# Parsoa/SVDSS

Measured on AMD Instinct MI355X. Metric: reads/sec through search+call, 30x HiFi 15 kb reads vs 3 Gb ref, 1/2/4/8 GPU, higher is better.
Workload: dtype int64

## Files before the change

svdss_amd/csrc/call_dp.hip:

```cpp
#include <hip/hip_runtime.h>

#include <cstdint>
#include <algorithm>
#include <chrono>
#include <cstdio>
#include <cstring>
#include <new>
#include <string>
#include <vector>

#include "../../include/svdss_hip.h"
#include "call_streams.h"
#include "dev_arena.h"
#include "hip_check.h"

#define DP_NEG (-0x20000000)
#define DP_THREADS 256

struct GapModel { int q, e, q2, e2; };

__device__ __forceinline__ int dp_gap(int l, const GapModel& g) {
  const int a = g.q + l * g.e, b = g.q2 + l * g.e2;
  return a < b ? a : b;
}

struct AlnPair {
  int64_t q_off, t_off;
  int64_t bnd_off;
  int64_t dir_off;
  int64_t cig_off;
  int32_t ql, tl;
  int32_t slot;
  int32_t waves;
};

__device__ __forceinline__ int dp_shr1(int x) {
  return __builtin_amdgcn_update_dpp(x, x, 0x138, 0xf, 0xf, false);
}

template <int W>
__global__ void __launch_bounds__(64 * W) align_wave_kernel(
    const AlnPair* pairs, const uint8_t* qsyms, const uint8_t* tsyms, int m, const int8_t* mat_g,
    GapModel gm, int32_t* ws, uint8_t* dirs, uint32_t* cigars, int32_t* scores, int32_t* n_cigar, int32_t* abort_flag) {
  const AlnPair P = pairs[blockIdx.x];
  const int ql = P.ql, tl = P.tl;
  const int lane = threadIdx.x & 63, wave = threadIdx.x >> 6;
  const int Wp = W > 1 ? P.waves : 1, NB = Wp + 1;
  if (wave >= Wp) return;
  if (ql <= 0 || tl <= 0) {
    if (lane == 0) { scores[P.slot] = 0; n_cigar[P.slot] = 0; }
    return;
  }
  __shared__ volatile int32_t prog[W + 1];
  __shared__ int32_t s_score;
  const uint8_t* q = qsyms + P.q_off;
  const uint8_t* t = tsyms + P.t_off;
  uint8_t* dir = dirs + P.dir_off;
  const int bstride = ql + 64;
  int32_t* bnd = ws + P.bnd_off;
  {
    int32_t* b0 = bnd + (int64_t)(NB - 1) * 3 * bstride;
    for (int j = threadIdx.x; j < ql; j += 64 * Wp) { b0[j] = -dp_gap(j + 1, gm); b0[bstride + j] = DP_NEG; b0[2 * bstride + j] = DP_NEG; }
    if ((int)threadIdx.x < NB) prog[threadIdx.x] = (int)threadIdx.x == NB - 1 ? ql : 0;
    __builtin_amdgcn_fence(__ATOMIC_RELEASE, "workgroup");
  }
  __syncthreads();
  const int n_stripes = (tl + 63) >> 6;
  int32_t final_score = 0;
  bool aborted = false;
  for (int s = wave; s < n_stripes && !aborted; s += Wp) {
    const int in_slot = (s + NB - 1) % NB, out_slot = s % NB;
    const int32_t* bin = bnd + (int64_t)in_slot * 3 * bstride;
    int32_t* bout = bnd + (int64_t)out_slot * 3 * bstride;
    if (W > 1 && lane == 0) prog[out_slot] = (s + 1) << 20;
    const int i = (s << 6) + lane;
    const bool row_ok = i < tl;
    const int rows = tl - (s << 6) < 64 ? tl - (s << 6) : 64;
    const bool writes_bnd = lane == 63 && s + 1 < n_stripes;
    uint64_t rowbits = 0;
    {
      const int ti = row_ok ? t[i] : 0;
      for (int k = 0; k < m; ++k) rowbits |= (uint64_t)(uint8_t)mat_g[ti * m + k] << (8 * k);
    }
    int32_t Hl = -dp_gap(i + 1, gm), Fl = DP_NEG, F2l = DP_NEG;
    int32_t Hout = 0, Eout = DP_NEG, E2out = DP_NEG;
    int32_t Hd = 0;
    int qcur = 0;
    const int n_steps = ql + rows - 1;
    int32_t nH = 0, nE = 0, nE2 = 0;
    int nq = 0;
    auto fetch = [&](int tau0) {
      const int jj = tau0 + lane;
      const bool in = jj < ql;
      nq = in ? q[jj] : 0;
      if (W > 1 && Wp > 1) {
        const int need = tau0 + 64 < ql ? tau0 + 64 : ql;
        int polls = 0;
        for (;;) {
          const int32_t v = prog[in_slot];
          if ((v >> 20) == s && (v & 0xFFFFF) >= need) break;
          if (++polls > (1 << 22)) { aborted = true; break; }
          __builtin_amdgcn_s_sleep(2);
        }
        if (aborted) { nH = 0; nE = 0; nE2 = 0; return; }
        __builtin_amdgcn_fence(__ATOMIC_ACQUIRE, "workgroup");
        nH = in ? __hip_atomic_load(&bin[jj], __ATOMIC_RELAXED, __HIP_MEMORY_SCOPE_WORKGROUP) : 0;
        nE = in ? __hip_atomic_load(&bin[bstride + jj], __ATOMIC_RELAXED, __HIP_MEMORY_SCOPE_WORKGROUP) : 0;
        nE2 = in ? __hip_atomic_load(&bin[2 * bstride + jj], __ATOMIC_RELAXED, __HIP_MEMORY_SCOPE_WORKGROUP) : 0;
      } else {
        nH = in ? bin[jj] : 0; nE = in ? bin[bstride + jj] : 0; nE2 = in ? bin[2 * bstride + jj] : 0;
      }
    };
    fetch(0);
    uint8_t* dcell = dir + (int64_t)(s << 6) * tl + i;
    for (int tau0 = 0; tau0 < n_steps && !aborted; tau0 += 64) {
      asm volatile("" : "+v"(nq), "+v"(nH), "+v"(nE), "+v"(nE2));
      const int qblk = nq;
      const int32_t bH = nH, bE = nE, bE2 = nE2;
      if (tau0 + 64 < n_steps) fetch(tau0 + 64);
      const int kmax = n_steps - tau0 < 64 ? n_steps - tau0 : 64;
      for (int k = 0; k < kmax; ++k) {
        const int tau = tau0 + k;
        const int qs = __builtin_amdgcn_readlane(qblk, k);
        const int32_t hb = __builtin_amdgcn_readlane(bH, k), eb = __builtin_amdgcn_readlane(bE, k),
                      e2b = __builtin_amdgcn_readlane(bE2, k);
        qcur = dp_shr1(qcur);
        int32_t Hu = dp_shr1(Hout), Eu = dp_shr1(Eout), E2u = dp_shr1(E2out);
        if (lane == 0) { qcur = qs; Hu = hb; Eu = eb; E2u = e2b; }
        const int j = tau - lane;
        if (row_ok && j >= 0 && j < ql) {
          const int32_t hdiag = j == 0 ? (i == 0 ? 0 : -dp_gap(i, gm)) : Hd;
          const int32_t Ein = (Hu - gm.q > Eu ? Hu - gm.q : Eu) - gm.e;
          const int32_t E2in = (Hu - gm.q2 > E2u ? Hu - gm.q2 : E2u) - gm.e2;
          const int32_t Fin = (Hl - gm.q > Fl ? Hl - gm.q : Fl) - gm.e;
          const int32_t F2in = (Hl - gm.q2 > F2l ? Hl - gm.q2 : F2l) - gm.e2;
          int32_t z = hdiag + (int32_t)(int8_t)(rowbits >> (8 * qcur));
          uint32_t d = 0;
          if (Ein > z) { d = 1; z = Ein; }
          if (Fin > z) { d = 2; z = Fin; }
          if (E2in > z) { d = 3; z = E2in; }
          if (F2in > z) { d = 4; z = F2in; }
          if (Ein > z - gm.q) d |= 0x08;
          if (Fin > z - gm.q) d |= 0x10;
          if (E2in > z - gm.q2) d |= 0x20;
          if (F2in > z - gm.q2) d |= 0x40;
          *dcell = (uint8_t)d;
          Hout = z; Eout = Ein; E2out = E2in;
          Hl = z; Fl = Fin; F2l = F2in;
          if (writes_bnd) { bout[j] = z; bout[bstride + j] = Ein; bout[2 * bstride + j] = E2in; }
          if (i == tl - 1 && j == ql - 1) final_score = z;
        }
        Hd = Hu;
        dcell += tl;
      }
      if (W > 1 && Wp > 1 && s + 1 < n_stripes) {
        __builtin_amdgcn_fence(__ATOMIC_RELEASE, "workgroup");
        const int done = tau0 + kmax - 63;
        if (lane == 63) prog[out_slot] = ((s + 1) << 20) | (done < 0 ? 0 : done > ql ? ql : done);
      }
    }
    if (W == 1 || Wp == 1) __syncthreads();
    else if (s + 1 < n_stripes) { __builtin_amdgcn_fence(__ATOMIC_RELEASE, "workgroup"); if (lane == 63) prog[out_slot] = ((s + 1) << 20) | ql; }
    if (s == n_stripes - 1) {
      const int owner = (tl - 1) & 63;
      final_score = __builtin_amdgcn_readlane(final_score, owner);
      if (lane == 0) s_score = final_score;
    }
  }
  if (aborted && lane == 0) atomicExch(abort_flag, 1);
  __syncthreads();
  if (wave != 0) return;
  final_score = s_score;
  {
    if (lane == 0) scores[P.slot] = final_score;
    uint32_t* cg = cigars + P.cig_off;
    int n = 0, i = tl - 1, j = ql - 1, state = 0;
    uint32_t cur_op = 0xffffffffu, cur_len = 0;
    auto push = [&](uint32_t op, uint32_t len) {
      if (op == cur_op) { cur_len += len; return; }
      if (cur_op != 0xffffffffu) { if (lane == 0) cg[n] = (cur_len << 4) | cur_op; ++n; }
      cur_op = op; cur_len = len;
    };
    int i0 = -(1 << 28), j0 = 0;
    uint32_t win = 0;
    while (i >= 0 && j >= 0) {
      int k = i0 - i, d = j - (j0 - k);
      if (k < 0 || k > 63 || d < 0 || d > 3) {
        i0 = i; j0 = j - 1; k = 0; d = 1;
        const int ii = i0 - lane;
        const int64_t jj = (int64_t)j0 - lane;
        win = 0;
        if (ii >= 0) {
#pragma unroll
          for (int x = 0; x < 4; ++x) {
            const int64_t c = jj + x;
            if (c >= 0 && c < ql) win |= (uint32_t)dir[(int64_t)(ii + c) * tl + ii] << (8 * x);
          }
        }
        asm volatile("" : "+v"(win));
      }
      const uint32_t tmp = ((uint32_t)__builtin_amdgcn_readlane((int)win, k) >> (8 * d)) & 0xffu;
      if (state == 0) state = tmp & 7;
      else if (!((tmp >> (state + 2)) & 1)) state = 0;
      if (state == 0) state = tmp & 7;
      if (state == 0) { push(0, 1); --i; --j; }
      else if (state == 1 || state == 3) { push(2, 1); --i; }
      else { push(1, 1); --j; }
    }
    if (i >= 0) push(2, (uint32_t)(i + 1));
    if (j >= 0) push(1, (uint32_t)(j + 1));
    if (cur_op != 0xffffffffu) { if (lane == 0) cg[n] = (cur_len << 4) | cur_op; ++n; }
    if (lane == 0) n_cigar[P.slot] = n;
  }
}

__device__ __forceinline__ void dp_lds_barrier() {
  __builtin_amdgcn_fence(__ATOMIC_RELEASE, "workgroup", "local");
  __builtin_amdgcn_s_barrier();
  __builtin_amdgcn_fence(__ATOMIC_ACQUIRE, "workgroup", "local");
}

struct LcsPair {
  int64_t a_off, b_off, ws_off;
  int32_t la, lb;
};

template <bool LDS>
__global__ void __launch_bounds__(DP_THREADS) lcs_ratio_kernel(const LcsPair* pairs, const uint8_t* as,
                                                              const uint8_t* bs, int32_t* ws,
                                                              int64_t* lcs_out, double* ratio_out) {
  extern __shared__ int32_t dp_lds[];
  const LcsPair P = pairs[blockIdx.x];
  const int la = P.la, lb = P.lb;
  int64_t lcs = 0;
  if (la > 0 && lb > 0) {
    const uint8_t* a = as + P.a_off;
    const uint8_t* b = bs + P.b_off;
    const int stride = la + 1;
    int32_t* buf = LDS ? dp_lds : ws + P.ws_off;
    if (LDS) {
      uint8_t* sa = (uint8_t*)(dp_lds + 3 * stride);
      uint8_t* sb = sa + la;
      for (int x = threadIdx.x; x < la; x += DP_THREADS) sa[x] = a[x];
      for (int x = threadIdx.x; x < lb; x += DP_THREADS) sb[x] = b[x];
      a = sa;
      b = sb;
      __syncthreads();
    }
    const int n_diag = la + lb - 1;
    for (int r = 0; r < n_diag; ++r) {
      const int32_t* Lm1 = buf + ((r + 2) % 3) * stride;
      const int32_t* Lm2 = buf + ((r + 1) % 3) * stride;
      int32_t* Lc = buf + (r % 3) * stride;
      const int ilo = r - (lb - 1) > 0 ? r - (lb - 1) : 0;
      const int ihi = r < la - 1 ? r : la - 1;
      for (int i = ilo + (int)threadIdx.x; i <= ihi; i += DP_THREADS) {
        const int j = r - i;
        const int32_t diag = (i > 0 && j > 0) ? Lm2[i - 1] : 0;
        const int32_t up = i > 0 ? Lm1[i - 1] : 0;
        const int32_t left = j > 0 ? Lm1[i] : 0;
        Lc[i] = a[i] == b[j] ? diag + 1 : (up > left ? up : left);
      }
      if (LDS) dp_lds_barrier(); else __syncthreads();
    }
    lcs = buf[((n_diag - 1) % 3) * stride + la - 1];
  }
  if (threadIdx.x == 0) {
    const int64_t maximum = (int64_t)la + lb;
    const int64_t dist = maximum - 2 * lcs;
    const double norm_dist = maximum ? (double)dist / (double)maximum : 0.0;
    const double norm_sim = 1.0 - norm_dist;
    lcs_out[blockIdx.x] = lcs;
    ratio_out[blockIdx.x] = norm_sim * 100.0;
  }
}

__global__ void __launch_bounds__(64) lcs_bits_kernel(const LcsPair* pairs, const uint8_t* as, const uint8_t* bs,
                                                      const uint8_t* sym_id, int64_t* lcs_out, double* ratio_out) {
  __shared__ unsigned long long pm[8][64];
  const LcsPair P = pairs[blockIdx.x];
  const int lane = threadIdx.x;
  const bool swap = P.la > P.lb;
  const uint8_t* pat = swap ? bs + P.b_off : as + P.a_off;
  const uint8_t* txt = swap ? as + P.a_off : bs + P.b_off;
  const int m = swap ? P.lb : P.la, n = swap ? P.la : P.lb;
  int64_t lcs = 0;
  if (m > 0) {
    unsigned long long mk[8] = {0, 0, 0, 0, 0, 0, 0, 0};
    for (int i = 0; i < 64; ++i) {
      const int pos = 64 * lane + i;
      const int id = pos < m ? (int)sym_id[pat[pos]] : 255;
#pragma unroll
      for (int k = 0; k < 8; ++k) mk[k] |= (unsigned long long)(id == k) << i;
    }
#pragma unroll
    for (int k = 0; k < 8; ++k) pm[k][lane] = mk[k];
    __syncthreads();
    unsigned long long V = ~0ull;
    for (int j0 = 0; j0 < n; j0 += 64) {
      const int tid = j0 + lane < n ? (int)sym_id[txt[j0 + lane]] : 255;
      const int cnt = n - j0 < 64 ? n - j0 : 64;
      int id = __builtin_amdgcn_readlane(tid, 0);
      unsigned long long cur = id < 8 ? pm[id][lane] : 0ull;
      for (int t = 0; t < cnt; ++t) {
        const int idn = __builtin_amdgcn_readlane(tid, t + 1 < cnt ? t + 1 : t);
        const unsigned long long nxt = idn < 8 ? pm[idn][lane] : 0ull;
        const unsigned long long U = V & cur;
        unsigned long long sum = V + U;
        const unsigned long long gen = __ballot(sum < V), pass = __ballot(sum == ~0ull);
        const unsigned long long carry = (pass + (gen << 1)) ^ pass;
        sum += (carry >> lane) & 1ull;
        V = sum | (V - U);
        cur = nxt;
      }
    }
    const int valid = m - 64 * lane;
    const unsigned long long vm = valid >= 64 ? ~0ull : valid <= 0 ? 0ull : ((1ull << valid) - 1);
    int z = (int)__popcll(~V & vm);
    for (int o = 32; o > 0; o >>= 1) z += __shfl_xor(z, o, 64);
    lcs = z;
  }
  if (lane == 0) {
    const int64_t maximum = (int64_t)P.la + P.lb;
    const int64_t dist = maximum - 2 * lcs;
    const double norm_dist = maximum ? (double)dist / (double)maximum : 0.0;
    const double norm_sim = 1.0 - norm_dist;
    lcs_out[blockIdx.x] = lcs;
    ratio_out[blockIdx.x] = norm_sim * 100.0;
  }
}


struct svdss_aln_batch {
  int64_t n_pairs = 0;
  int64_t total_cigar = 0;
  int64_t cells = 0;
  double kernel_ms = 0.0;
  int64_t info[4] = {0, 0, 0, 0};
  std::vector<int32_t> scores;
  std::vector<int64_t> n_cigar;
  std::vector<uint32_t> cigar;
  int device = -1;
  DevArena arena;
};

namespace {
struct DevMem {
  void* p = nullptr;
  ~DevMem() { if (p) (void)hipFree(p); }
  int alloc(size_t bytes) {
    HIPCHK(hipMalloc(&p, bytes ? bytes : 16));
    return SVDSS_OK;
  }
};
}

extern "C" int svdss_align_global_batch(const uint8_t* queries, const int64_t* q_off,
                                        const uint8_t* targets, const int64_t* t_off, int64_t n_pairs,
                                        int32_t m, const int8_t* mat, int32_t gapo, int32_t gape,
                                        int32_t gapo2, int32_t gape2, int32_t device,
                                        svdss_aln_batch_t** out) {
  if (!out || n_pairs < 0 || m < 1 || m > 8 || !mat || device < 0) return SVDSS_EINVAL;
  if (n_pairs > 0 && (!queries || !q_off || !targets || !t_off)) return SVDSS_EINVAL;
  HIPCHK(hipSetDevice(device));
  svdss_aln_batch* b = *out ? *out : new (std::nothrow) svdss_aln_batch();
  if (!b) return SVDSS_ENOMEM;
  *out = b;
  b->n_pairs = n_pairs;
  b->total_cigar = 0;
  b->cells = 0;
  b->kernel_ms = 0.0;
  b->info[0] = b->info[1] = b->info[2] = b->info[3] = 0;
  b->scores.assign((size_t)n_pairs, 0);
  b->n_cigar.assign((size_t)n_pairs, 0);
  b->cigar.clear();
  if (n_pairs == 0) return SVDSS_OK;
  for (int64_t i = 0; i < n_pairs; ++i) {
    const int64_t ql = q_off[i + 1] - q_off[i], tl = t_off[i + 1] - t_off[i];
    if (ql < 0 || tl < 0) return SVDSS_EINVAL;
    if (ql >= (1 << 28) || tl >= (1 << 28)) return SVDSS_ERANGE;
  }
  const int64_t qtot = q_off[n_pairs] - q_off[0], ttot = t_off[n_pairs] - t_off[0];
  if (b->device != device) {
    b->arena.drop();
    b->device = device;
  }
  CallStreamLease lease;
  HIPCHK(lease.acquire(device));
  const hipStream_t st = lease.get();
  const GapModel gm{gapo, gape, gapo2, gape2};
  hipEvent_t ev0, ev1;
  HIPCHK(hipEventCreate(&ev0));
  HIPCHK(hipEventCreate(&ev1));
  int64_t dir_budget = (int64_t)24 << 30;
  {
    size_t free_b = 0, total_b = 0;
    if (hipMemGetInfo(&free_b, &total_b) == hipSuccess)
      dir_budget = std::min<int64_t>(dir_budget, (int64_t)((free_b + b->arena.cap) / 2));
    if (dir_budget < ((int64_t)1 << 30)) dir_budget = (int64_t)1 << 30;
    if (getenv("SVDSS_ALIGN_DIR_MB") && atoll(getenv("SVDSS_ALIGN_DIR_MB")) > 0) dir_budget = atoll(getenv("SVDSS_ALIGN_DIR_MB")) << 20;
  }
  std::vector<int32_t> h_nc((size_t)n_pairs, 0);
  std::vector<std::pair<int64_t, int64_t>> cig_at((size_t)n_pairs);
  std::vector<std::vector<uint32_t>> chunk_cigs;
  int64_t start = 0;
  const int ALN_W = getenv("SVDSS_ALIGN_WAVES") && atoi(getenv("SVDSS_ALIGN_WAVES")) == 8 ? 8 : 4;
  const int64_t aln_frac = getenv("SVDSS_ALIGN_FRAC") && atoll(getenv("SVDSS_ALIGN_FRAC")) > 0 ? atoll(getenv("SVDSS_ALIGN_FRAC")) : 8;
  int64_t max_cells = 0;
  for (int64_t i = 0; i < n_pairs; ++i) max_cells = std::max(max_cells, (q_off[i + 1] - q_off[i]) * (t_off[i + 1] - t_off[i]));
  bool multi = !(getenv("SVDSS_ALIGN_WAVES") && atoi(getenv("SVDSS_ALIGN_WAVES")) <= 1);
  auto waves_of = [&](int64_t ql, int64_t tl) {
    if (!multi || tl < 8 * 64 || ql >= (1 << 20)) return 1;
    return (ql * tl * aln_frac >= max_cells || n_pairs < 2048) ? ALN_W : 1;
  };
  while (start < n_pairs) {
    std::vector<AlnPair> hp;
    int64_t ws = 0, dirb = 0, cig = 0, end = start;
    bool any_multi = false;
    while (end < n_pairs) {
      const int64_t ql = q_off[end + 1] - q_off[end], tl = t_off[end + 1] - t_off[end];
      const int64_t need = (ql + tl) * tl;
      if (end > start && dirb + need > dir_budget) break;
      AlnPair a;
      memset(&a, 0, sizeof a);
      a.q_off = q_off[end] - q_off[0];
      a.t_off = t_off[end] - t_off[0];
      a.bnd_off = ws;
      a.dir_off = dirb;
      a.cig_off = cig;
      a.ql = (int32_t)ql;
      a.tl = (int32_t)tl;
      a.slot = (int32_t)(end - start);
      a.waves = waves_of(ql, tl);
      any_multi = any_multi || a.waves > 1;
      hp.push_back(a);
      cig_at[(size_t)end] = {cig, (int64_t)chunk_cigs.size()};
      ws += 3 * (a.waves + 1) * (ql + 64);
      dirb += need;
      cig += ql + tl + 2;
      b->cells += ql * tl;
      ++end;
    }
    const int64_t np = end - start;
    std::stable_sort(hp.begin(), hp.end(), [](const AlnPair& x, const AlnPair& y) {
      return (int64_t)x.ql * x.tl > (int64_t)y.ql * y.tl;
    });
    const size_t need_bytes = DevArena::padded((size_t)qtot) + DevArena::padded((size_t)ttot) + DevArena::padded(64) +
                              DevArena::padded(sizeof(AlnPair) * (size_t)np) + DevArena::padded(sizeof(int32_t) * (size_t)ws) +
                              DevArena::padded((size_t)dirb) + DevArena::padded(sizeof(uint32_t) * (size_t)cig) +
                              2 * DevArena::padded(sizeof(int32_t) * (size_t)np) + DevArena::padded(64);
    HIPCHK(b->arena.reserve(need_bytes));
    void* d_q = b->arena.take((size_t)qtot);
    void* d_t = b->arena.take((size_t)ttot);
    void* d_mat = b->arena.take(64);
    void* d_pairs = b->arena.take(sizeof(AlnPair) * (size_t)np);
    void* d_ws = b->arena.take(sizeof(int32_t) * (size_t)ws);
    void* d_dir = b->arena.take((size_t)dirb);
    void* d_cig = b->arena.take(sizeof(uint32_t) * (size_t)cig);
    void* d_sc = b->arena.take(sizeof(int32_t) * (size_t)np);
    void* d_nc = b->arena.take(sizeof(int32_t) * (size_t)np);
    void* d_abort = b->arena.take(64);
    if (qtot) HIPCHK(hipMemcpyAsync(d_q, queries + q_off[0], (size_t)qtot, hipMemcpyHostToDevice, st));
    if (ttot) HIPCHK(hipMemcpyAsync(d_t, targets + t_off[0], (size_t)ttot, hipMemcpyHostToDevice, st));
    HIPCHK(hipMemcpyAsync(d_mat, mat, (size_t)(m * m), hipMemcpyHostToDevice, st));
    HIPCHK(hipMemcpyAsync(d_pairs, hp.data(), sizeof(AlnPair) * (size_t)np, hipMemcpyHostToDevice, st));
    HIPCHK(hipMemsetAsync(d_abort, 0, 64, st));
    HIPCHK(hipEventRecord(ev0, st));
    if (any_multi && ALN_W == 8)
      hipLaunchKernelGGL(align_wave_kernel<8>, dim3((unsigned)np), dim3(64 * 8), 0, st, (const AlnPair*)d_pairs,
                         (const uint8_t*)d_q, (const uint8_t*)d_t, (int)m, (const int8_t*)d_mat, gm, (int32_t*)d_ws,
                         (uint8_t*)d_dir, (uint32_t*)d_cig, (int32_t*)d_sc, (int32_t*)d_nc, (int32_t*)d_abort);
    else if (any_multi)
      hipLaunchKernelGGL(align_wave_kernel<4>, dim3((unsigned)np), dim3(64 * 4), 0, st, (const AlnPair*)d_pairs,
                         (const uint8_t*)d_q, (const uint8_t*)d_t, (int)m, (const int8_t*)d_mat, gm, (int32_t*)d_ws,
                         (uint8_t*)d_dir, (uint32_t*)d_cig, (int32_t*)d_sc, (int32_t*)d_nc, (int32_t*)d_abort);
    else
      hipLaunchKernelGGL(align_wave_kernel<1>, dim3((unsigned)np), dim3(64), 0, st, (const AlnPair*)d_pairs,
                         (const uint8_t*)d_q, (const uint8_t*)d_t, (int)m, (const int8_t*)d_mat, gm, (int32_t*)d_ws,
                         (uint8_t*)d_dir, (uint32_t*)d_cig, (int32_t*)d_sc, (int32_t*)d_nc, (int32_t*)d_abort);
    HIPCHK(hipGetLastError());
    HIPCHK(hipEventRecord(ev1, st));
    if (any_multi) {
      int32_t ab = 0;
      HIPCHK(hipMemcpyAsync(&ab, d_abort, sizeof ab, hipMemcpyDeviceToHost, st));
      HIPCHK(hipStreamSynchronize(st));
      if (ab) {
        fprintf(stderr, "[svdss] realignment: a multi-wavefront pair did not finish; the batch runs again with one wavefront per pair\n");
        multi = false;
        ++b->info[3];
        b->cells -= [&] { int64_t c = 0; for (const AlnPair& a : hp) c += (int64_t)a.ql * a.tl; return c; }();
        for (int64_t k = start; k < end; ++k) cig_at[(size_t)k] = {0, 0};
        continue;
      }
    }
    ++b->info[0];
    for (const AlnPair& a : hp) b->info[1] += a.waves > 1;
    b->info[2] = std::max<int64_t>(b->info[2], any_multi ? ALN_W : 1);
    chunk_cigs.emplace_back((size_t)cig);
    HIPCHK(hipMemcpyAsync(&b->scores[(size_t)start], d_sc, sizeof(int32_t) * (size_t)np, hipMemcpyDeviceToHost, st));
    HIPCHK(hipMemcpyAsync(&h_nc[(size_t)start], d_nc, sizeof(int32_t) * (size_t)np, hipMemcpyDeviceToHost, st));
    if (cig) HIPCHK(hipMemcpyAsync(chunk_cigs.back().data(), d_cig, sizeof(uint32_t) * (size_t)cig, hipMemcpyDeviceToHost, st));
    HIPCHK(hipStreamSynchronize(st));
    float ms = 0.f;
    HIPCHK(hipEventElapsedTime(&ms, ev0, ev1));
    b->kernel_ms += ms;
    start = end;
  }
  {
    int64_t total = 0;
    for (int64_t k = 0; k < n_pairs; ++k) total += h_nc[(size_t)k];
    b->cigar.resize((size_t)total);
    int64_t o = 0;
    for (int64_t k = 0; k < n_pairs; ++k) {
      const int32_t nc = h_nc[(size_t)k];
      b->n_cigar[(size_t)k] = nc;
      const uint32_t* src = chunk_cigs[(size_t)cig_at[(size_t)k].second].data() + cig_at[(size_t)k].first;
      for (int x = nc - 1; x >= 0; --x) b->cigar[(size_t)o++] = src[x];
    }
  }
  (void)hipEventDestroy(ev0);
  (void)hipEventDestroy(ev1);
  b->total_cigar = (int64_t)b->cigar.size();
  return SVDSS_OK;
}

extern "C" int64_t svdss_aln_batch_npairs(const svdss_aln_batch_t* b) { return b ? b->n_pairs : -1; }
extern "C" int64_t svdss_aln_batch_total_cigar(const svdss_aln_batch_t* b) { return b ? b->total_cigar : -1; }
extern "C" int64_t svdss_aln_batch_cells(const svdss_aln_batch_t* b) { return b ? b->cells : -1; }
extern "C" double svdss_aln_batch_kernel_ms(const svdss_aln_batch_t* b) { return b ? b->kernel_ms : -1.0; }

extern "C" int svdss_aln_batch_launch_info(const svdss_aln_batch_t* b, int64_t out[4]) {
  if (!b || !out) return SVDSS_EINVAL;
  memcpy(out, b->info, sizeof b->info);
  return SVDSS_OK;
}

extern "C" int svdss_aln_batch_fetch(const svdss_aln_batch_t* b, int32_t* scores, int64_t* n_cigar,
                                     uint32_t* cigar) {
  if (!b) return SVDSS_EINVAL;
  if (scores) memcpy(scores, b->scores.data(), sizeof(int32_t) * b->scores.size());
  if (n_cigar) memcpy(n_cigar, b->n_cigar.data(), sizeof(int64_t) * b->n_cigar.size());
  if (cigar) memcpy(cigar, b->cigar.data(), sizeof(uint32_t) * b->cigar.size());
  return SVDSS_OK;
}

extern "C" void svdss_aln_batch_free(svdss_aln_batch_t* b) { delete b; }

static thread_local int32_t g_ratio_last_kernel = -1;
extern "C" int32_t svdss_indel_ratio_last_kernel(void) { return g_ratio_last_kernel; }

extern "C" int svdss_indel_ratio_batch(const uint8_t* a, const int64_t* a_off, const uint8_t* bsy,
                                       const int64_t* b_off, int64_t n_pairs, int32_t device,
                                       double* ratio_out, int64_t* lcs_out) {
  if (n_pairs < 0 || device < 0) return SVDSS_EINVAL;
  if (n_pairs == 0) return SVDSS_OK;
  if (!a || !a_off || !bsy || !b_off || !ratio_out) return SVDSS_EINVAL;
  HIPCHK(hipSetDevice(device));
  std::vector<LcsPair> hp((size_t)n_pairs);
  int64_t ws = 0, la_max = 0, lb_max = 0;
  for (int64_t i = 0; i < n_pairs; ++i) {
    const int64_t la = a_off[i + 1] - a_off[i], lb = b_off[i + 1] - b_off[i];
    if (la < 0 || lb < 0) return SVDSS_EINVAL;
    if (la >= (1 << 30) || lb >= (1 << 30)) return SVDSS_ERANGE;
    hp[(size_t)i].a_off = a_off[i] - a_off[0];
    hp[(size_t)i].b_off = b_off[i] - b_off[0];
    hp[(size_t)i].ws_off = ws;
    hp[(size_t)i].la = (int32_t)la;
    hp[(size_t)i].lb = (int32_t)lb;
    ws += 3 * (la + 1);
    if (la > la_max) la_max = la;
    if (lb > lb_max) lb_max = lb;
  }
  const int64_t atot = a_off[n_pairs] - a_off[0], btot = b_off[n_pairs] - b_off[0];
  struct RatioState {
    int device = -1;
    DevArena arena;
  };
  static thread_local RatioState R;
  if (R.device != device) {
    R.arena.drop();
    R.device = device;
  }
  CallStreamLease lease;
  HIPCHK(lease.acquire(device));
  const hipStream_t st = lease.get();
  HIPCHK(R.arena.reserve(DevArena::padded((size_t)atot) + DevArena::padded((size_t)btot) +
                          DevArena::padded(sizeof(LcsPair) * (size_t)n_pairs) + DevArena::padded(sizeof(int32_t) * (size_t)ws) +
                          DevArena::padded(sizeof(int64_t) * (size_t)n_pairs) + DevArena::padded(sizeof(double) * (size_t)n_pairs) +
                          DevArena::padded(256)));
  struct { void* p; } d_a{R.arena.take((size_t)atot)}, d_b{R.arena.take((size_t)btot)},
      d_pairs{R.arena.take(sizeof(LcsPair) * (size_t)n_pairs)}, d_ws{R.arena.take(sizeof(int32_t) * (size_t)ws)},
      d_lcs{R.arena.take(sizeof(int64_t) * (size_t)n_pairs)}, d_ratio{R.arena.take(sizeof(double) * (size_t)n_pairs)};
  if (atot) HIPCHK(hipMemcpyAsync(d_a.p, a + a_off[0], (size_t)atot, hipMemcpyHostToDevice, st));
  if (btot) HIPCHK(hipMemcpyAsync(d_b.p, bsy + b_off[0], (size_t)btot, hipMemcpyHostToDevice, st));
  HIPCHK(hipMemcpyAsync(d_pairs.p, hp.data(), sizeof(LcsPair) * (size_t)n_pairs, hipMemcpyHostToDevice, st));
  bool bits_ok = !getenv("SVDSS_RATIO_DP");
  uint8_t sym_id[256];
  if (bits_ok) {
    for (int64_t i = 0; i < n_pairs && bits_ok; ++i) bits_ok = std::min(hp[(size_t)i].la, hp[(size_t)i].lb) <= 4096;
    uint8_t any = 0;
    for (int64_t i = 0; i < atot; ++i) any |= a[a_off[0] + i];
    for (int64_t i = 0; i < btot; ++i) any |= bsy[b_off[0] + i];
    memset(sym_id, 255, sizeof sym_id);
    if (any < 8) {
      for (int k = 0; k < 8; ++k) sym_id[k] = (uint8_t)k;
    } else if (bits_ok) {
      bool seen[256] = {false};
      for (int64_t i = 0; i < atot; ++i) seen[a[a_off[0] + i]] = true;
      for (int64_t i = 0; i < btot; ++i) seen[bsy[b_off[0] + i]] = true;
      int nd = 0;
      for (int c = 0; c < 256; ++c)
        if (seen[c]) { if (nd < 8) sym_id[c] = (uint8_t)nd; ++nd; }
      if (nd > 8) bits_ok = false;
    }
  }
  if (bits_ok) {
    void* d_map = R.arena.take(256);
    HIPCHK(hipMemcpyAsync(d_map, sym_id, 256, hipMemcpyHostToDevice, st));
    g_ratio_last_kernel = 0;
    hipLaunchKernelGGL(lcs_bits_kernel, dim3((unsigned)n_pairs), dim3(64), 0, st, (const LcsPair*)d_pairs.p,
                       (const uint8_t*)d_a.p, (const uint8_t*)d_b.p, (const uint8_t*)d_map, (int64_t*)d_lcs.p, (double*)d_ratio.p);
    HIPCHK(hipGetLastError());
    HIPCHK(hipMemcpyAsync(ratio_out, d_ratio.p, sizeof(double) * (size_t)n_pairs, hipMemcpyDeviceToHost, st));
    if (lcs_out) HIPCHK(hipMemcpyAsync(lcs_out, d_lcs.p, sizeof(int64_t) * (size_t)n_pairs, hipMemcpyDeviceToHost, st));
    HIPCHK(hipStreamSynchronize(st));
    return SVDSS_OK;
  }
  const size_t lds_need = sizeof(int32_t) * 3 * (size_t)(la_max + 1) + (size_t)la_max + (size_t)lb_max + 16;
  if (lds_need <= 150 * 1024) {
    HIPCHK(hipFuncSetAttribute((const void*)lcs_ratio_kernel<true>, hipFuncAttributeMaxDynamicSharedMemorySize, (int)lds_need));
    g_ratio_last_kernel = 1;
    hipLaunchKernelGGL(lcs_ratio_kernel<true>, dim3((unsigned)n_pairs), dim3(DP_THREADS), lds_need, st,
                       (const LcsPair*)d_pairs.p, (const uint8_t*)d_a.p, (const uint8_t*)d_b.p, (int32_t*)d_ws.p,
                       (int64_t*)d_lcs.p, (double*)d_ratio.p);
  } else {
    g_ratio_last_kernel = 2;
    hipLaunchKernelGGL(lcs_ratio_kernel<false>, dim3((unsigned)n_pairs), dim3(DP_THREADS), 0, st,
                       (const LcsPair*)d_pairs.p, (const uint8_t*)d_a.p, (const uint8_t*)d_b.p, (int32_t*)d_ws.p,
                       (int64_t*)d_lcs.p, (double*)d_ratio.p);
  }
  HIPCHK(hipGetLastError());
  HIPCHK(hipMemcpyAsync(ratio_out, d_ratio.p, sizeof(double) * (size_t)n_pairs, hipMemcpyDeviceToHost, st));
  if (lcs_out) HIPCHK(hipMemcpyAsync(lcs_out, d_lcs.p, sizeof(int64_t) * (size_t)n_pairs, hipMemcpyDeviceToHost, st));
  HIPCHK(hipStreamSynchronize(st));
  return SVDSS_OK;
}
```

svdss_amd/csrc/poa.hip:

```cpp
#include <hip/hip_runtime.h>

#include <algorithm>
#include <chrono>
#include <cstdint>
#include <cstdio>
#include <cstdlib>
#include <cstring>
#include <new>
#include <string>
#include <vector>

#include "../../include/svdss_hip.h"
#include "call_streams.h"
#include "dev_arena.h"
#include "hip_check.h"
#include "poa_plan.h"
#include "poa_wave.h"
#include "poa_quad.h"

#define PNEG (-0x20000000)
#define P_O1 4
#define P_E1 2
#define P_O2 24
#define P_E2 1
#define P_MATCH 2
#define P_MISMATCH 4

struct PoaGraph {
  int n_nodes, n_edges, cap_nodes, cap_edges;
  uint8_t* base;
  int *out_head, *out_tail, *in_head, *in_tail, *order, *index, *deg, *best, *row_beg, *row_end, *mpl, *mpr, *aln;
  int *e_from, *e_to, *e_w, *e_next_out, *e_next_in;
  int64_t *row_off, *score;
};

__device__ __forceinline__ int p_score(int a, int b) { return (a >= 4 || b >= 4) ? 0 : (a == b ? P_MATCH : -P_MISMATCH); }

__device__ int g_new_node(PoaGraph& g, int base) {
  const int v = g.n_nodes++;
  g.base[v] = (uint8_t)base;
  g.out_head[v] = g.out_tail[v] = g.in_head[v] = g.in_tail[v] = -1;
  for (int b = 0; b < 5; ++b) g.aln[5 * v + b] = -1;
  return v;
}

__device__ void g_add_edge(PoaGraph& g, int u, int v) {
  for (int e = g.out_head[u]; e >= 0; e = g.e_next_out[e])
    if (g.e_to[e] == v) { g.e_w[e]++; return; }
  const int e = g.n_edges++;
  g.e_from[e] = u; g.e_to[e] = v; g.e_w[e] = 1;
  g.e_next_out[e] = -1; g.e_next_in[e] = -1;
  if (g.out_tail[u] < 0) g.out_head[u] = e; else g.e_next_out[g.out_tail[u]] = e;
  g.out_tail[u] = e;
  if (g.in_tail[v] < 0) g.in_head[v] = e; else g.e_next_in[g.in_tail[v]] = e;
  g.in_tail[v] = e;
}

__device__ void g_toposort(PoaGraph& g) {
  for (int v = 0; v < g.n_nodes; ++v) g.deg[v] = 0;
  for (int e = 0; e < g.n_edges; ++e) g.deg[g.e_to[e]]++;
  int qh = 0, qt = 0;
  g.order[qt++] = 0;
  while (qh < qt) {
    const int u = g.order[qh];
    g.index[u] = qh++;
    for (int e = g.out_head[u]; e >= 0; e = g.e_next_out[e])
      if (--g.deg[g.e_to[e]] == 0) g.order[qt++] = g.e_to[e];
  }
}

struct PoaDp { int32_t *H, *Hp, *E1, *E2, *F1, *F2; };

__device__ __forceinline__ int32_t dp_at(const int32_t* arr, const PoaGraph& g, int r, int j) {
  return (j < g.row_beg[r] || j > g.row_end[r]) ? PNEG : arr[g.row_off[r] + (j - g.row_beg[r])];
}

__device__ __forceinline__ int32_t wave_scan_max(int32_t x, int lane) {
#pragma unroll
  for (int d = 1; d < 64; d <<= 1) {
    const int32_t y = __shfl_up(x, d, 64);
    if (lane >= d && y > x) x = y;
  }
  return x;
}

__device__ bool poa_forward(PoaGraph& g, const PoaDp& dp, const uint8_t* q, int L, int w, int64_t pool_cap,
                            unsigned long long& cells) {
  const int lane = threadIdx.x & 63;
  const int n = g.n_nodes;
  int64_t used = 0;
  for (int r = 0; r < n; ++r) {
    const int v = g.order[r];
    if (v == 1) {
      if (lane == 0) { g.row_beg[r] = 0; g.row_end[r] = -1; g.row_off[r] = used; g.mpl[r] = 0; g.mpr[r] = 0; }
      __syncthreads();
      continue;
    }
    int beg, end;
    if (r == 0) { beg = 0; end = w < L ? w : L; }
    else {
      int lo = 1 << 30, hi = -1;
      for (int e = g.in_head[v]; e >= 0; e = g.e_next_in[e]) {
        const int ur = g.index[g.e_from[e]];
        const int a = g.mpl[ur], b = g.mpr[ur];
        if (a < lo) lo = a;
        if (b > hi) hi = b;
      }
      beg = lo + 1 - w; if (beg < 0) beg = 0;
      end = hi + 1 + w; if (end > L) end = L;
      if (end - beg + 1 > 2 * w + 129) end = beg + 2 * w + 128;
    }
    const int width = end - beg + 1;
    if (used + width > pool_cap) return false;
    if (lane == 0) { g.row_beg[r] = beg; g.row_end[r] = end; g.row_off[r] = used; }
    const int64_t off = used;
    used += width;
    int32_t best = PNEG; int mpl = beg, mpr = beg;
    int32_t g1 = PNEG, g2 = PNEG;
    for (int j0 = beg; j0 <= end; j0 += 64) {
      const int j = j0 + lane;
      const bool in = j <= end;
      int32_t m = PNEG, e1 = PNEG, e2 = PNEG;
      if (in) {
        if (r == 0) m = (j == 0) ? 0 : PNEG;
        else {
          const int bv = g.base[v];
          for (int e = g.in_head[v]; e >= 0; e = g.e_next_in[e]) {
            const int ur = g.index[g.e_from[e]];
            if (j >= 1) {
              const int32_t h = dp_at(dp.H, g, ur, j - 1);
              if (h > PNEG / 2) { const int32_t x = h + p_score(bv, q[j - 1]); if (x > m) m = x; }
            }
            const int32_t h = dp_at(dp.H, g, ur, j);
            {
              const int32_t x = dp_at(dp.E1, g, ur, j);
              const int32_t a = h > PNEG / 2 ? h - P_O1 : PNEG, b = x > PNEG / 2 ? x : PNEG;
              int32_t c = a > b ? a : b;
              if (c > PNEG / 2) { c -= P_E1; if (c > e1) e1 = c; }
            }
            {
              const int32_t x = dp_at(dp.E2, g, ur, j);
              const int32_t a = h > PNEG / 2 ? h - P_O2 : PNEG, b = x > PNEG / 2 ? x : PNEG;
              int32_t c = a > b ? a : b;
              if (c > PNEG / 2) { c -= P_E2; if (c > e2) e2 = c; }
            }
          }
        }
      }
      int32_t hp = m; if (e1 > hp) hp = e1; if (e2 > hp) hp = e2;
      const int32_t t1 = (in && hp > PNEG / 2) ? hp + j * P_E1 : PNEG;
      const int32_t t2 = (in && hp > PNEG / 2) ? hp + j * P_E2 : PNEG;
      const int32_t s1 = wave_scan_max(t1, lane), s2 = wave_scan_max(t2, lane);
      int32_t x1 = __shfl_up(s1, 1, 64), x2 = __shfl_up(s2, 1, 64);
      if (lane == 0) { x1 = PNEG; x2 = PNEG; }
      if (g1 > x1) x1 = g1;
      if (g2 > x2) x2 = g2;
      const int32_t f1 = x1 > PNEG / 2 ? x1 - P_O1 - j * P_E1 : PNEG;
      const int32_t f2 = x2 > PNEG / 2 ? x2 - P_O2 - j * P_E2 : PNEG;
      int32_t h = hp; if (f1 > h) h = f1; if (f2 > h) h = f2;
      if (in) {
        const int64_t o = off + (j - beg);
        dp.Hp[o] = hp; dp.E1[o] = e1; dp.E2[o] = e2; dp.F1[o] = f1; dp.F2[o] = f2; dp.H[o] = h;
      }
      const int32_t c1 = __shfl(s1, 63, 64), c2 = __shfl(s2, 63, 64);
      if (c1 > g1) g1 = c1;
      if (c2 > g2) g2 = c2;
      int32_t hm = in ? h : PNEG;
#pragma unroll
      for (int d = 32; d >= 1; d >>= 1) { const int32_t y = __shfl_xor(hm, d, 64); if (y > hm) hm = y; }
      const unsigned long long eq = __ballot(in && h == hm);
      if (eq) {
        const int l = j0 + __builtin_ctzll(eq), rr = j0 + 63 - __builtin_clzll(eq);
        if (hm > best) { best = hm; mpl = l; mpr = rr; }
        else if (hm == best) mpr = rr;
      }
    }
    if (lane == 0) { g.mpl[r] = mpl; g.mpr[r] = mpr; }
    cells += (unsigned long long)width;
    __syncthreads();
  }
  return true;
}

__device__ int poa_traceback(const PoaGraph& g, const PoaDp& dp, const uint8_t* q, int L, int* op_node, int* op_q) {
  int bu = -1; int32_t bs = PNEG;
  for (int e = g.in_head[1]; e >= 0; e = g.e_next_in[e]) {
    const int32_t h = dp_at(dp.H, g, g.index[g.e_from[e]], L);
    if (h > bs) { bs = h; bu = g.e_from[e]; }
  }
  if (bu < 0 || bs <= PNEG / 2) return -1;
  int nops = 0, v = bu, j = L, state = 0;
  while (v != 0 || j > 0) {
    const int r = g.index[v];
    if (v == 0) { op_node[nops] = -1; op_q[nops] = j - 1; ++nops; --j; continue; }
    if (state == 0 || state == 5) {
      const int32_t h = state == 0 ? dp_at(dp.H, g, r, j) : dp_at(dp.Hp, g, r, j);
      bool moved = false;
      if (j >= 1) {
        for (int e = g.in_head[v]; e >= 0 && !moved; e = g.e_next_in[e]) {
          const int u = g.e_from[e];
          const int32_t x = dp_at(dp.H, g, g.index[u], j - 1);
          if (x > PNEG / 2 && x + p_score(g.base[v], q[j - 1]) == h) {
            op_node[nops] = v; op_q[nops] = j - 1; ++nops; v = u; --j; state = 0; moved = true;
          }
        }
      }
      if (moved) continue;
      if (dp_at(dp.E1, g, r, j) == h) { state = 1; continue; }
      if (dp_at(dp.E2, g, r, j) == h) { state = 2; continue; }
      if (state == 0 && dp_at(dp.F1, g, r, j) == h) { state = 3; continue; }
      if (state == 0 && dp_at(dp.F2, g, r, j) == h) { state = 4; continue; }
      return -1;
    } else if (state == 1 || state == 2) {
      const int32_t* E = state == 1 ? dp.E1 : dp.E2;
      const int o = state == 1 ? P_O1 : P_O2, ee = state == 1 ? P_E1 : P_E2;
      const int32_t x = dp_at(E, g, r, j);
      bool moved = false;
      for (int e = g.in_head[v]; e >= 0 && !moved; e = g.e_next_in[e]) {
        const int u = g.e_from[e];
        const int32_t h = dp_at(dp.H, g, g.index[u], j);
        if (h > PNEG / 2 && h - o - ee == x) { op_node[nops] = v; op_q[nops] = -1; ++nops; v = u; state = 0; moved = true; }
      }
      for (int e = g.in_head[v]; e >= 0 && !moved; e = g.e_next_in[e]) {
        const int u = g.e_from[e];
        const int32_t y = dp_at(E, g, g.index[u], j);
        if (y > PNEG / 2 && y - ee == x) { op_node[nops] = v; op_q[nops] = -1; ++nops; v = u; moved = true; }
      }
      if (!moved) return -1;
    } else {
      const int32_t* F = state == 3 ? dp.F1 : dp.F2;
      const int o = state == 3 ? P_O1 : P_O2, ee = state == 3 ? P_E1 : P_E2;
      const int32_t x = dp_at(F, g, r, j);
      op_node[nops] = -1; op_q[nops] = j - 1; ++nops;
      const int32_t hp = dp_at(dp.Hp, g, r, j - 1);
      if (hp > PNEG / 2 && hp - o - ee == x) state = 5;
      --j;
    }
  }
  return nops;
}

__global__ void __launch_bounds__(64) poa_consensus_kernel(const PoaTask* tasks, const uint8_t* seqs, const int64_t* seq_off,
                                                          int32_t* ws32, int64_t* ws64, uint8_t* ws8,
                                                          int32_t* cons_len, int32_t* status, unsigned long long* cells) {
  const PoaTask T = tasks[blockIdx.x];
  const int lane = threadIdx.x;
  __shared__ int sh_flag;
  PoaGraph g;
  g.cap_nodes = T.cap_nodes; g.cap_edges = T.cap_edges; g.n_nodes = 0; g.n_edges = 0;
  int32_t* nb = ws32 + T.node_off;
  const int64_t cn = T.cap_nodes, ce = T.cap_edges;
  g.out_head = nb; g.out_tail = nb + cn; g.in_head = nb + 2 * cn; g.in_tail = nb + 3 * cn;
  g.order = nb + 4 * cn; g.index = nb + 5 * cn; g.deg = nb + 6 * cn; g.best = nb + 7 * cn;
  g.row_beg = nb + 8 * cn; g.row_end = nb + 9 * cn; g.mpl = nb + 10 * cn; g.mpr = nb + 11 * cn; g.aln = nb + 12 * cn;
  int32_t* eb = ws32 + T.edge_off;
  g.e_from = eb; g.e_to = eb + ce; g.e_w = eb + 2 * ce; g.e_next_out = eb + 3 * ce; g.e_next_in = eb + 4 * ce;
  g.row_off = ws64 + T.row_off64; g.score = ws64 + T.row_off64 + cn;
  g.base = ws8 + T.base_off;
  PoaDp dp;
  int32_t* db = ws32 + T.dp_off;
  dp.H = db; dp.Hp = db + T.pool_cap; dp.E1 = db + 2 * T.pool_cap; dp.E2 = db + 3 * T.pool_cap;
  dp.F1 = db + 4 * T.pool_cap; dp.F2 = db + 5 * T.pool_cap;
  int* op_node = ws32 + T.op_off;
  int* op_q = op_node + (T.cap_nodes + T.max_len + 4);
  uint8_t* cons = ws8 + T.cons_off;
  const int n = (int)T.n_seqs;
  if (n <= 0) { if (lane == 0) { cons_len[blockIdx.x] = 0; status[blockIdx.x] = 0; } return; }
  __shared__ int sh_nodes, sh_edges;
  unsigned long long my_cells = 0;
  if (lane == 0) {
    g_new_node(g, 4); g_new_node(g, 4);
    const uint8_t* q = seqs + seq_off[T.seq_first];
    const int L = (int)(seq_off[T.seq_first + 1] - seq_off[T.seq_first]);
    int last = 0;
    for (int j = 0; j < L; ++j) { const int v = g_new_node(g, q[j]); g.aln[5 * v + q[j]] = v; g_add_edge(g, last, v); last = v; }
    g_add_edge(g, last, 1);
    sh_nodes = g.n_nodes; sh_edges = g.n_edges;
  }
  __syncthreads();
  g.n_nodes = sh_nodes; g.n_edges = sh_edges;
  for (int i = 1; i < n; ++i) {
    const uint8_t* q = seqs + seq_off[T.seq_first + i];
    const int L = (int)(seq_off[T.seq_first + i + 1] - seq_off[T.seq_first + i]);
    if (lane == 0) g_toposort(g);
    __syncthreads();
    int w = 10 + (int)(0.01 * L);
    int nops = -1;
    for (int attempt = 0; attempt < 2; ++attempt) {
      const bool fit = poa_forward(g, dp, q, L, w, T.pool_cap, my_cells);
      if (!fit) { if (lane == 0) status[blockIdx.x] = 1; return; }
      if (lane == 0) sh_flag = poa_traceback(g, dp, q, L, op_node, op_q);
      __syncthreads();
      nops = sh_flag;
      __syncthreads();
      if (nops >= 0) break;
      w = L;
    }
    if (nops < 0) { if (lane == 0) status[blockIdx.x] = 2; return; }
    if (lane == 0) {
      int last = 0;
      for (int k = nops - 1; k >= 0; --k) {
        const int v = op_node[k], j = op_q[k];
        if (v >= 0 && j >= 0) {
          int use;
          if (g.base[v] == q[j]) use = v;
          else if (g.aln[5 * v + q[j]] >= 0) use = g.aln[5 * v + q[j]];
          else {
            use = g_new_node(g, q[j]);
            for (int b = 0; b < 5; ++b) {
              const int sib = g.aln[5 * v + b];
              g.aln[5 * use + b] = sib;
              if (sib >= 0) g.aln[5 * sib + q[j]] = use;
            }
            g.aln[5 * use + q[j]] = use;
          }
          g_add_edge(g, last, use); last = use;
        } else if (v < 0) {
          const int use = g_new_node(g, q[j]);
          g.aln[5 * use + q[j]] = use;
          g_add_edge(g, last, use); last = use;
        }
      }
      g_add_edge(g, last, 1);
      sh_nodes = g.n_nodes; sh_edges = g.n_edges;
    }
    __syncthreads();
    g.n_nodes = sh_nodes; g.n_edges = sh_edges;
  }
  if (lane == 0) {
    g_toposort(g);
    for (int r = g.n_nodes - 1; r >= 0; --r) {
      const int v = g.order[r];
      int bst = -1, bw = -1; int64_t bsc = -1;
      for (int e = g.out_head[v]; e >= 0; e = g.e_next_out[e]) {
        const int x = g.e_to[e];
        if (g.e_w[e] > bw || (g.e_w[e] == bw && g.score[x] > bsc)) { bw = g.e_w[e]; bsc = g.score[x]; bst = x; }
      }
      g.best[v] = bst;
      g.score[v] = bst >= 0 ? bw + bsc : 0;
    }
    int len = 0;
    for (int v = g.best[0]; v >= 0 && v != 1; v = g.best[v]) cons[len++] = g.base[v];
    cons_len[blockIdx.x] = len;
    status[blockIdx.x] = 0;
    atomicAdd(cells, my_cells);
  }
}


struct svdss_poa_batch {
  int64_t n_clusters = 0;
  int64_t n_hbm = 0;
  int64_t n_quad_back = 0;
  int64_t cells = 0;
  double kernel_ms = 0.0;
  std::vector<int64_t> cons_len;
  std::vector<uint8_t> cons;
  int device = -1;
  DevArena in_arena, ws_arena;
};

static_assert(poa_padded(0) == DevArena::padded(0) && poa_padded(1001) == DevArena::padded(1001), "poa_plan.h sizes what ws_arena hands out");

namespace {
struct EventPair {
  hipEvent_t a = nullptr, b = nullptr;
  int create() {
    if (!a) HIPCHK(hipEventCreate(&a));
    if (!b) HIPCHK(hipEventCreate(&b));
    return SVDSS_OK;
  }
  ~EventPair() { if (a) (void)hipEventDestroy(a); if (b) (void)hipEventDestroy(b); }
};

struct PoaBatchRun {
  svdss_poa_batch& b;
  const uint8_t* seqs;
  PoaBatchIn in;
  void *d_seqs = nullptr, *d_off = nullptr, *d_cells = nullptr;
  CallStreamLease lease;
  hipStream_t s0 = nullptr;
  EventPair ev;
  std::vector<std::vector<uint8_t>> results;
  std::vector<int64_t> todo;
  std::vector<uint8_t> round0_no_wider, skip_round0;
  struct Mem { void *tasks, *w32, *w64, *w8, *len, *st; };

  PoaBatchRun(svdss_poa_batch& batch, const uint8_t* s, const int64_t* seq_off, const int64_t* cluster_off, int64_t n_clusters)
      : b(batch), seqs(s), results((size_t)n_clusters), round0_no_wider((size_t)n_clusters, 0), skip_round0((size_t)n_clusters, 0) {
    in.seq_off = seq_off; in.cluster_off = cluster_off; in.n_clusters = n_clusters;
    in.knobs = PoaKnobs::from_env();
  }

  int upload(int32_t device) {
    const int64_t n_seqs_total = in.cluster_off[in.n_clusters];
    const int64_t total_syms = in.seq_off[n_seqs_total];
    for (int64_t i = 0; i < n_seqs_total; ++i) {
      const int64_t l = in.seq_off[i + 1] - in.seq_off[i];
      if (l < 0) return SVDSS_EINVAL;
      if (l >= (1 << 24)) return SVDSS_ERANGE;
    }
    if (total_syms > 0 && !seqs) return SVDSS_EINVAL;
    if (b.device != device) {
      b.in_arena.drop(); b.ws_arena.drop();
      b.device = device;
    }
    const size_t off_bytes = sizeof(int64_t) * (size_t)(n_seqs_total + 1);
    HIPCHK(b.in_arena.reserve(DevArena::padded((size_t)total_syms) + DevArena::padded(off_bytes) + DevArena::padded(8)));
    d_seqs = b.in_arena.take((size_t)total_syms); d_off = b.in_arena.take(off_bytes); d_cells = b.in_arena.take(8);
    HIPCHK(lease.acquire(device));
    s0 = lease.get();
    if (total_syms) HIPCHK(hipMemcpyAsync(d_seqs, seqs, (size_t)total_syms, hipMemcpyHostToDevice, s0));
    HIPCHK(hipMemcpyAsync(d_off, in.seq_off, off_bytes, hipMemcpyHostToDevice, s0));
    HIPCHK(hipMemsetAsync(d_cells, 0, 8, s0));
    hipDeviceProp_t prop;
    if (hipGetDeviceProperties(&prop, device) == hipSuccess && prop.multiProcessorCount > 0) in.n_cus = prop.multiProcessorCount;
    size_t free_b = 0, total_b = 0;
    const bool have = hipMemGetInfo(&free_b, &total_b) == hipSuccess;
    in.ws_budget = poa_ws_budget(in.knobs, have, free_b, b.ws_arena.cap);
    in.set_max_work();
    return SVDSS_OK;
  }

  bool empty(int64_t c) const { return in.cluster_off[c + 1] == in.cluster_off[c]; }

  Mem take(size_t task_bytes, size_t nt, int64_t w32, int64_t w64, int64_t w8) {
    Mem m;
    m.tasks = b.ws_arena.take(task_bytes * nt);
    m.w32 = b.ws_arena.take(sizeof(int32_t) * (size_t)w32);
    m.w64 = w64 ? b.ws_arena.take(sizeof(int64_t) * (size_t)w64) : nullptr;
    m.w8 = b.ws_arena.take((size_t)w8);
    m.len = b.ws_arena.take(sizeof(int32_t) * nt);
    m.st = b.ws_arena.take(sizeof(int32_t) * nt);
    return m;
  }

  int rounds() {
    std::vector<int64_t> cur((size_t)in.n_clusters), next;
    for (int64_t c = 0; c < in.n_clusters; ++c) cur[(size_t)c] = c;
    for (int round = in.knobs.use_quad ? -1 : 0; round < kPoaRounds && !cur.empty(); ++round) {
      const PoaRoundPlan p = poa_plan_round(in, round, cur, skip_round0, round0_no_wider);
      next = p.next;
      for (int64_t c : p.hbm) { todo.push_back(c); if (!empty(c)) ++b.n_hbm; }
      for (size_t w = 0; w + 1 < p.cuts.size(); ++w)
        if (const int rc = run_wave(round, p, p.cuts[w], p.cuts[w + 1], next)) return rc;
      cur.swap(next);
      if (round < 0) std::sort(cur.begin(), cur.end());
    }
    std::sort(todo.begin(), todo.end());
    return SVDSS_OK;
  }

  int run_wave(int round, const PoaRoundPlan& p, size_t g0, size_t g1, std::vector<int64_t>& next) {
    const bool quad = round < 0;
    size_t tot_bytes = 0;
    for (size_t gi = g0; gi < g1; ++gi) tot_bytes += p.groups[gi].bytes();
    const auto ta = std::chrono::steady_clock::now();
    HIPCHK(b.ws_arena.reserve(tot_bytes));
    const double as = std::chrono::duration<double>(std::chrono::steady_clock::now() - ta).count();
    if (in.knobs.debug && as > 0.005) fprintf(stderr, "[poa] workspace of %.1f GB taken in %.3f s\n", (double)tot_bytes / 1073741824.0, as);
    const std::vector<PoaLaunch> launches = poa_merge_wave(in.knobs, p.groups, g0, g1);
    struct Unit { const PoaGroup* g; PoaGroup merged; size_t n2 = 0; int max_len2 = 0, max_len1 = 0; bool pair = false; Mem m; };
    std::vector<Unit> units(launches.size());
    for (size_t k = 0; k < launches.size(); ++k) {
      const PoaLaunch& L = launches[k];
      Unit& u = units[k];
      if (L.single >= 0) u.g = &p.groups[(size_t)L.single];
      else {
        const PoaGroup *c2 = L.c2 >= 0 ? &p.groups[(size_t)L.c2] : nullptr, *c1 = L.c1 >= 0 ? &p.groups[(size_t)L.c1] : nullptr;
        u.pair = true;
        u.merged = poa_merged_group(c2, c1, u.n2);
        u.max_len2 = c2 ? c2->max_len : 0;
        u.max_len1 = c1 ? c1->max_len : 0;
      }
    }
    for (Unit& u : units) {
      if (u.pair) u.g = &u.merged;
      const size_t nt = u.g->tasks.size();
      u.m = take(sizeof(PoaWaveTask), nt, u.g->w32, 0, u.g->w8);
      HIPCHK(hipMemcpyAsync(u.m.tasks, u.g->tasks.data(), sizeof(PoaWaveTask) * nt, hipMemcpyHostToDevice, s0));
      HIPCHK(hipMemsetAsync(u.m.st, 0xff, sizeof(int32_t) * nt, s0));
    }
    std::vector<CallStreamLease> side(units.empty() ? 0 : std::min<size_t>(units.size() - 1, 5));
    for (CallStreamLease& l : side) HIPCHK(l.acquire(b.device, true));
    if (!side.empty()) HIPCHK(hipStreamSynchronize(s0));
    const auto t0 = std::chrono::steady_clock::now();
    for (size_t k = 0; k < units.size(); ++k) {
      const Unit& u = units[k];
      const PoaGroup& g = *u.g;
      const Mem& m = u.m;
      const size_t si = k % (side.size() + 1);
      const hipStream_t gs = si ? side[si - 1].get() : s0;
      const PoaWaveTask* d_tasks = (const PoaWaveTask*)m.tasks;
      const int nt = (int)g.tasks.size();
      if (u.pair) {
        HIPCHK(poa_quad_pair_launch(d_tasks, (int)u.n2, nt - (int)u.n2, u.max_len2, u.max_len1, (const uint8_t*)d_seqs, (const int64_t*)d_off,
                                     (int32_t*)m.w32, (int32_t*)m.len, (int32_t*)m.st, (unsigned long long*)d_cells, gs));
        HIPCHK(poa_bundle_launch(d_tasks, nt, g.bundle_lds, (int32_t*)m.w32, (uint8_t*)m.w8, (int32_t*)m.len, (const int32_t*)m.st, gs));
        if (u.n2 && (size_t)nt > u.n2) { std::lock_guard<std::mutex> lock(call_stream_pool().mu); ++call_stream_pool().merged; }
      } else if (g.gw) {
        HIPCHK(poa_quad_launch(g.gw, g.cols, d_tasks, nt, g.max_len, (const uint8_t*)d_seqs, (const int64_t*)d_off, (int32_t*)m.w32,
                                (int32_t*)m.len, (int32_t*)m.st, (unsigned long long*)d_cells, gs));
        HIPCHK(poa_bundle_launch(d_tasks, nt, g.bundle_lds, (int32_t*)m.w32, (uint8_t*)m.w8, (int32_t*)m.len, (const int32_t*)m.st, gs));
      } else
        HIPCHK(poa_wave_launch(g.cols, d_tasks, nt, g.lds, g.bundle_lds, (const uint8_t*)d_seqs, (const int64_t*)d_off, (int32_t*)m.w32,
                                (uint8_t*)m.w8, (int32_t*)m.len, (int32_t*)m.st, (unsigned long long*)d_cells, gs));
    }
    for (CallStreamLease& l : side) HIPCHK(hipStreamSynchronize(l.get()));
    HIPCHK(hipStreamSynchronize(s0));
    side.clear();
    const double ms = std::chrono::duration<double, std::milli>(std::chrono::steady_clock::now() - t0).count();
    b.kernel_ms += ms;
    int why[8] = {0, 0, 0, 0, 0, 0, 0, 0};
    int64_t n_run = 0;
    for (const Unit& u : units) {
      n_run += (int64_t)u.g->tasks.size();
      if (const int rc = collect(round, u.g->tasks, u.g->ids, u.m, u.g->w8, next, why)) return rc;
    }
    if (in.knobs.debug) {
      if (quad) poa_quad_debug_report(); else poa_wave_debug_report();
      fprintf(stderr, "[poa] %s round %d: %lld clusters in %zu launches, %.3f ms, not done: first-read %d preds %d width %d band %d capacity %d other %d\n",
              quad ? "quad" : "wave", round, (long long)n_run, units.size(), ms, why[1], why[2], why[3], why[4], why[5], why[0] + why[6] + why[7]);
    }
    return SVDSS_OK;
  }

  template <class Task>
  int collect(int stage, const std::vector<Task>& tasks, const std::vector<int64_t>& ids, const Mem& m, int64_t w8, std::vector<int64_t>& next, int* why) {
    const size_t nt = tasks.size();
    std::vector<int32_t> lens(nt), st(nt);
    std::vector<uint8_t> h8((size_t)w8);
    HIPCHK(hipMemcpyAsync(lens.data(), m.len, sizeof(int32_t) * nt, hipMemcpyDeviceToHost, s0));
    HIPCHK(hipMemcpyAsync(st.data(), m.st, sizeof(int32_t) * nt, hipMemcpyDeviceToHost, s0));
    if (w8) HIPCHK(hipMemcpyAsync(h8.data(), m.w8, (size_t)w8, hipMemcpyDeviceToHost, s0));
    HIPCHK(hipStreamSynchronize(s0));
    for (size_t k = 0; k < nt; ++k) {
      const int64_t id = ids[k];
      if (st[k] == 0) {
        const uint8_t* src = h8.data() + tasks[k].cons_off;
        results[(size_t)id].assign(src, src + lens[k]);
        continue;
      }
      const int reason = (st[k] >> 8) & 7;
      ++why[reason];
      if (stage < 0) {
        next.push_back(id);
        ++b.n_quad_back;
        if (reason == 3 && round0_no_wider[(size_t)id]) skip_round0[(size_t)id] = 1;
      } else if (stage + 1 < kPoaRounds && (reason == 3 || reason == 4 || reason == 5)) next.push_back(id);
      else if (stage < kPoaRounds) { todo.push_back(id); ++b.n_hbm; }
      else if (stage == kPoaRounds && st[k] == 1) next.push_back(id);
      else return SVDSS_ERANGE;
    }
    return SVDSS_OK;
  }

  int fallback() {
    for (int pass = 0; pass < 2 && !todo.empty(); ++pass) {
      std::vector<int64_t> next;
      PoaHbmLaunch L;
      for (size_t pos = 0; pos < todo.size();) {
        pos = poa_plan_hbm(in.seq_off, in.cluster_off, todo, pos, pass, L);
        const size_t nt = L.tasks.size();
        HIPCHK(b.ws_arena.reserve(poa_padded(sizeof(PoaTask) * nt) + poa_padded(sizeof(int32_t) * (size_t)L.w32) + poa_padded(sizeof(int64_t) * (size_t)L.w64) +
                                  poa_padded((size_t)L.w8) + 2 * poa_padded(sizeof(int32_t) * nt)));
        const Mem m = take(sizeof(PoaTask), nt, L.w32, L.w64, L.w8);
        HIPCHK(hipMemcpyAsync(m.tasks, L.tasks.data(), sizeof(PoaTask) * nt, hipMemcpyHostToDevice, s0));
        HIPCHK(hipMemsetAsync(m.st, 0xff, sizeof(int32_t) * nt, s0));
        if (const int rc = ev.create()) return rc;
        HIPCHK(hipEventRecord(ev.a, s0));
        hipLaunchKernelGGL(poa_consensus_kernel, dim3((unsigned)nt), dim3(64), 0, s0, (const PoaTask*)m.tasks, (const uint8_t*)d_seqs,
                           (const int64_t*)d_off, (int32_t*)m.w32, (int64_t*)m.w64, (uint8_t*)m.w8, (int32_t*)m.len, (int32_t*)m.st,
                           (unsigned long long*)d_cells);
        HIPCHK(hipGetLastError());
        HIPCHK(hipEventRecord(ev.b, s0));
        HIPCHK(hipStreamSynchronize(s0));
        float ms = 0.f;
        HIPCHK(hipEventElapsedTime(&ms, ev.a, ev.b));
        b.kernel_ms += ms;
        int why[8] = {0, 0, 0, 0, 0, 0, 0, 0};
        if (const int rc = collect(kPoaRounds + pass, L.tasks, L.ids, m, L.w8, next, why)) return rc;
      }
      todo.swap(next);
    }
    return SVDSS_OK;
  }

  int gather() {
    unsigned long long cells = 0;
    HIPCHK(hipMemcpyAsync(&cells, d_cells, 8, hipMemcpyDeviceToHost, s0));
    HIPCHK(hipStreamSynchronize(s0));
    b.cells = (int64_t)cells;
    for (int64_t c = 0; c < in.n_clusters; ++c) {
      b.cons_len[(size_t)c] = (int64_t)results[(size_t)c].size();
      b.cons.insert(b.cons.end(), results[(size_t)c].begin(), results[(size_t)c].end());
    }
    return SVDSS_OK;
  }
};
}

extern "C" int svdss_poa_consensus_batch(const uint8_t* seqs, const int64_t* seq_off, const int64_t* cluster_off,
                                         int64_t n_clusters, int32_t device, svdss_poa_batch_t** out) {
  if (!out || n_clusters < 0 || device < 0) return SVDSS_EINVAL;
  if (n_clusters > 0 && (!seq_off || !cluster_off)) return SVDSS_EINVAL;
  HIPCHK(hipSetDevice(device));
  svdss_poa_batch* b = *out ? *out : new (std::nothrow) svdss_poa_batch();
  if (!b) return SVDSS_ENOMEM;
  *out = b;
  b->n_clusters = n_clusters;
  b->cells = 0;
  b->n_hbm = 0;
  b->n_quad_back = 0;
  b->kernel_ms = 0.0;
  b->cons_len.assign((size_t)n_clusters, 0);
  b->cons.clear();
  if (n_clusters == 0) return SVDSS_OK;
  PoaBatchRun run(*b, seqs, seq_off, cluster_off, n_clusters);
  int rc;
  if ((rc = run.upload(device)) || (rc = run.rounds()) || (rc = run.fallback())) return rc;
  return run.gather();
}

extern "C" int64_t svdss_poa_batch_nclusters(const svdss_poa_batch_t* b) { return b ? b->n_clusters : -1; }
extern "C" int64_t svdss_poa_batch_total(const svdss_poa_batch_t* b) { return b ? (int64_t)b->cons.size() : -1; }
extern "C" int64_t svdss_poa_batch_cells(const svdss_poa_batch_t* b) { return b ? b->cells : -1; }
extern "C" double svdss_poa_batch_kernel_ms(const svdss_poa_batch_t* b) { return b ? b->kernel_ms : -1.0; }
extern "C" int64_t svdss_poa_batch_hbm(const svdss_poa_batch_t* b) { return b ? b->n_hbm : -1; }
extern "C" int64_t svdss_poa_batch_quad_back(const svdss_poa_batch_t* b) { return b ? b->n_quad_back : -1; }
extern "C" int svdss_poa_batch_fetch(const svdss_poa_batch_t* b, int64_t* cons_len, uint8_t* cons) {
  if (!b) return SVDSS_EINVAL;
  if (cons_len) memcpy(cons_len, b->cons_len.data(), sizeof(int64_t) * b->cons_len.size());
  if (cons) memcpy(cons, b->cons.data(), b->cons.size());
  return SVDSS_OK;
}
extern "C" void svdss_poa_batch_free(svdss_poa_batch_t* b) { delete b; }

extern "C" int svdss_call_side_stat(int32_t device, int64_t out[4]) {
  if (!out || device < 0 || device >= kCallStreamDevices) return SVDSS_EINVAL;
  CallStreamPool& p = call_stream_pool();
  std::lock_guard<std::mutex> lock(p.mu);
  out[0] = p.live[device];
  out[1] = p.created;
  out[2] = p.merged;
  out[3] = p.borrowed;
  return SVDSS_OK;
}
```

svdss_amd/csrc/poa_quad.h:

```cpp
#pragma once
#include <hip/hip_runtime.h>

#include <cstddef>
#include <cstdint>

#include "poa_task.h"

hipError_t poa_quad_launch(int gw, int cols, const PoaWaveTask* d_tasks, int n_tasks, int max_len, const uint8_t* d_seqs, const int64_t* d_seq_off,
                           int32_t* ws32, int32_t* d_len, int32_t* d_status, unsigned long long* d_cells, hipStream_t stream);
hipError_t poa_quad_pair_launch(const PoaWaveTask* d_tasks, int n2, int n1, int max_len2, int max_len1, const uint8_t* d_seqs,
                                const int64_t* d_seq_off, int32_t* ws32, int32_t* d_len, int32_t* d_status, unsigned long long* d_cells,
                                hipStream_t stream);
void poa_quad_debug_report();
```

svdss_amd/csrc/poa_quad.hip:

```cpp
#include <hip/hip_runtime.h>

#include <algorithm>
#include <cstdint>
#include <cstdio>
#include <cstring>

#include "poa_plan.h"
#include "poa_quad.h"
#include "poa_quad_gfx950.h"
#include "poa_quad_core.h"

#ifndef PQ_MIN_WAVES
#define PQ_MIN_WAVES 1
#endif
template <int GW, int C>
__global__ void __launch_bounds__(64, PQ_MIN_WAVES) poa_quad_kernel(const PoaWaveTask* tasks, int n_tasks, const uint8_t* seqs, const int64_t* seq_off,
                                                      int32_t* ws32, int32_t* cons_len, int32_t* status, unsigned long long* cells, int qcap) {
  extern __shared__ __align__(16) int32_t poaq_lds[];
  pq::poaq_run<GW, C>(tasks, n_tasks, seqs, seq_off, ws32, cons_len, status, cells, poaq_lds, (int)blockIdx.x, qcap);
}

template <int GW, int C>
static hipError_t launch_gc(const PoaWaveTask* d_tasks, int n_tasks, int max_len, const uint8_t* d_seqs, const int64_t* d_seq_off, int32_t* ws32,
                            int32_t* d_len, int32_t* d_status, unsigned long long* d_cells, hipStream_t stream) {
  constexpr int G = 64 / GW;
  const size_t lds = pq::Geom<GW, C>::lds_bytes(max_len);
  if (lds > 160 * 1024 - 512) return hipErrorInvalidValue;
  hipError_t e = hipFuncSetAttribute((const void*)poa_quad_kernel<GW, C>, hipFuncAttributeMaxDynamicSharedMemorySize, (int)lds);
  if (e != hipSuccess) return e;
  hipLaunchKernelGGL((poa_quad_kernel<GW, C>), dim3((unsigned)((n_tasks + G - 1) / G)), dim3(64), lds, stream, d_tasks, n_tasks, d_seqs,
                     d_seq_off, ws32, d_len, d_status, d_cells, pq::Geom<GW, C>::qcap(max_len));
  return hipGetLastError();
}

__global__ void __launch_bounds__(64, PQ_MIN_WAVES) poa_quad_pair_kernel(const PoaWaveTask* tasks, int n2, int n1, const uint8_t* seqs,
                                                                         const int64_t* seq_off, int32_t* ws32, int32_t* cons_len, int32_t* status,
                                                                         unsigned long long* cells, int qcap2, int qcap1) {
  extern __shared__ __align__(16) int32_t poaq_lds[];
  const int block = (int)blockIdx.x;
  if (block < n2) pq::poaq_run<64, 2>(tasks, n2, seqs, seq_off, ws32, cons_len, status, cells, poaq_lds, block, qcap2);
  else pq::poaq_run<64, 1>(tasks + n2, n1, seqs, seq_off, ws32, cons_len + n2, status + n2, cells, poaq_lds, block - n2, qcap1);
}

hipError_t poa_quad_pair_launch(const PoaWaveTask* d_tasks, int n2, int n1, int max_len2, int max_len1, const uint8_t* d_seqs,
                                const int64_t* d_seq_off, int32_t* ws32, int32_t* d_len, int32_t* d_status, unsigned long long* d_cells,
                                hipStream_t stream) {
  if (n2 < 0 || n1 < 0 || n2 + n1 <= 0) return hipErrorInvalidValue;
  size_t lds = 0;
  if (n2) lds = std::max(lds, pq::Geom<64, 2>::lds_bytes(max_len2));
  if (n1) lds = std::max(lds, pq::Geom<64, 1>::lds_bytes(max_len1));
  if (lds > 160 * 1024 - 512) return hipErrorInvalidValue;
  hipError_t e = hipFuncSetAttribute((const void*)poa_quad_pair_kernel, hipFuncAttributeMaxDynamicSharedMemorySize, (int)lds);
  if (e != hipSuccess) return e;
  hipLaunchKernelGGL(poa_quad_pair_kernel, dim3((unsigned)(n2 + n1)), dim3(64), lds, stream, d_tasks, n2, n1, d_seqs, d_seq_off, ws32, d_len,
                     d_status, d_cells, pq::Geom<64, 2>::qcap(max_len2), pq::Geom<64, 1>::qcap(max_len1));
  return hipGetLastError();
}

hipError_t poa_quad_launch(int gw, int cols, const PoaWaveTask* d_tasks, int n_tasks, int max_len, const uint8_t* d_seqs, const int64_t* d_seq_off,
                           int32_t* ws32, int32_t* d_len, int32_t* d_status, unsigned long long* d_cells, hipStream_t stream) {
#define PQ_CASE(GW_, C_) \
  if (gw == GW_ && cols == C_) return launch_gc<GW_, C_>(d_tasks, n_tasks, max_len, d_seqs, d_seq_off, ws32, d_len, d_status, d_cells, stream)
  PQ_CASE(16, 3); PQ_CASE(16, 4); PQ_CASE(16, 5); PQ_CASE(16, 6); PQ_CASE(16, 7);
  PQ_CASE(32, 2); PQ_CASE(32, 3); PQ_CASE(32, 4);
  PQ_CASE(64, 1); PQ_CASE(64, 2);
#undef PQ_CASE
  return hipErrorInvalidValue;
}

void poa_quad_debug_report() {
  unsigned long long h[8];
  if (hipMemcpyFromSymbol(h, HIP_SYMBOL(pq::g_poaq_prof), sizeof h) != hipSuccess) return;
  fprintf(stderr, "[poa_quad] 100MHz ticks (sum over wavefronts): prepare %llu forward %llu traceback %llu update %llu | row steps %llu, %llu the general way\n",
          h[0], h[1], h[2], h[3], h[4], h[5]);
  memset(h, 0, sizeof h);
  (void)hipMemcpyToSymbol(HIP_SYMBOL(pq::g_poaq_prof), h, sizeof h);
}

template <int GW>
__device__ void selftest_gw(const int32_t* in, int32_t* out) {
  typedef pq::Grp<GW> GR;
  const int lane = (int)threadIdx.x;
  const int x = in[lane];
  int32_t* o = out + lane * 12;
  o[0] = GR::shr1(x, -7, 0);
  o[1] = GR::shl1(x, -9, 0);
  o[2] = GR::scan_max(x, 0);
  o[3] = GR::scan_add(x, 0);
  o[4] = GR::all_max(x, 0);
  o[5] = GR::all_min(x, 0);
  o[6] = GR::last(x, 0);
  o[7] = GR::from(x, (GR::last(x, 0) >> 3) & (GW - 1), 0);
  const uint64_t b = GR::bits((x & 1) != 0, 0);
  o[8] = (int32_t)(uint32_t)b;
  o[9] = (int32_t)(uint32_t)(b >> 32);
  o[10] = pq::wave_any(x == 12345, 0) ? 1 : 0;
  o[11] = pq::ctz64(~(b >> (lane % GW)));
}

__global__ void __launch_bounds__(64) poa_quad_selftest_kernel(const int32_t* in, int32_t* out) {
  selftest_gw<16>(in, out);
  selftest_gw<32>(in, out + 64 * 12);
  selftest_gw<64>(in, out + 2 * 64 * 12);
}

extern "C" int svdss_poa_quad_selftest(const int32_t* in, int32_t* out, int32_t device) {
  if (!in || !out || device < 0) return -1;
  if (hipSetDevice(device) != hipSuccess) return -2;
  int32_t *d_in = nullptr, *d_out = nullptr;
  if (hipMalloc(&d_in, 64 * 4) != hipSuccess || hipMalloc(&d_out, 3 * 64 * 12 * 4) != hipSuccess) return -3;
  int rc = 0;
  if (hipMemcpy(d_in, in, 64 * 4, hipMemcpyHostToDevice) != hipSuccess) rc = -4;
  if (!rc) {
    hipLaunchKernelGGL(poa_quad_selftest_kernel, dim3(1), dim3(64), 0, 0, d_in, d_out);
    if (hipDeviceSynchronize() != hipSuccess) rc = -5;
  }
  if (!rc && hipMemcpy(out, d_out, 3 * 64 * 12 * 4, hipMemcpyDeviceToHost) != hipSuccess) rc = -6;
  (void)hipFree(d_in); (void)hipFree(d_out);
  return rc;
}
```

svdss_amd/csrc/poa_wave.h:

```cpp
#pragma once
#include <hip/hip_runtime.h>

#include <cstddef>
#include <cstdint>

#include "poa_task.h"

hipError_t poa_wave_launch(int cols, const PoaWaveTask* d_tasks, int n_tasks, size_t lds_bytes, size_t bundle_lds_bytes,
                           const uint8_t* d_seqs, const int64_t* d_seq_off, int32_t* ws32, uint8_t* ws8, int32_t* d_len,
                           int32_t* d_status, unsigned long long* d_cells, hipStream_t stream);
hipError_t poa_bundle_launch(const PoaWaveTask* d_tasks, int n_tasks, size_t bundle_lds_bytes, int32_t* ws32, uint8_t* ws8, int32_t* d_len,
                             const int32_t* d_status, hipStream_t stream);
void poa_wave_debug_report();
```

svdss_amd/csrc/poa_wave.hip:

```cpp
#include <hip/hip_runtime.h>

#include <cstdint>
#include <cstdio>
#include <cstdlib>
#include <cstring>

#include "poa_plan.h"
#include "poa_wave.h"

#define PNEG (-0x20000000)
#define UNI(x) __builtin_amdgcn_readfirstlane(x)
#define TG 16
#define TGB 0x20000000
#define TG_M 15
#define TG_E1 7
#define TG_E2 6
#define TG_F1 5
#define TG_F2 4
#define P_O1 4
#define P_E1 2
#define P_O2 24
#define P_E2 1
#define P_MATCH 2
#define P_MISMATCH 4
#define COL_SINK 0x7FFFFFFE
#define COL_NEW 0x7FFFFFFF
#define RI_SLOW 3u

__device__ __forceinline__ int tg_up(int x, int tag) { return x <= PNEG / 2 ? 0 : (int)(((unsigned)x << 4) | (unsigned)tag) + TGB; }
__device__ __forceinline__ int tg_down(int x) { return x <= TGB / 2 ? PNEG : (x - TGB) >> 4; }
__device__ __forceinline__ int pl_score(int a, int b) { return (a >= 4 || b >= 4) ? 0 : (a == b ? P_MATCH : -P_MISMATCH); }
__device__ __forceinline__ int imax(int a, int b) { return a > b ? a : b; }
__device__ __forceinline__ int imin(int a, int b) { return a < b ? a : b; }

template <int CTRL, int RMASK>
__device__ __forceinline__ int dppi(int old, int src) {
  return __builtin_amdgcn_update_dpp(old, src, CTRL, RMASK, 0xf, false);
}

__device__ __forceinline__ int wave_scan_max(int x, int ident) {
  x = imax(x, dppi<0x111, 0xf>(ident, x));
  x = imax(x, dppi<0x112, 0xf>(ident, x));
  x = imax(x, dppi<0x114, 0xf>(ident, x));
  x = imax(x, dppi<0x118, 0xf>(ident, x));
  x = imax(x, dppi<0x142, 0xa>(ident, x));
  x = imax(x, dppi<0x143, 0xc>(ident, x));
  return x;
}

__device__ __forceinline__ int wave_scan_min(int x, int ident) {
  x = imin(x, dppi<0x111, 0xf>(ident, x));
  x = imin(x, dppi<0x112, 0xf>(ident, x));
  x = imin(x, dppi<0x114, 0xf>(ident, x));
  x = imin(x, dppi<0x118, 0xf>(ident, x));
  x = imin(x, dppi<0x142, 0xa>(ident, x));
  x = imin(x, dppi<0x143, 0xc>(ident, x));
  return x;
}

__device__ __forceinline__ int wave_scan_add(int x) {
  x += dppi<0x111, 0xf>(0, x);
  x += dppi<0x112, 0xf>(0, x);
  x += dppi<0x114, 0xf>(0, x);
  x += dppi<0x118, 0xf>(0, x);
  x += dppi<0x142, 0xa>(0, x);
  x += dppi<0x143, 0xc>(0, x);
  return x;
}

__device__ __forceinline__ int wave_shr1(int x, int fill) { return dppi<0x138, 0xf>(fill, x); }
__device__ __forceinline__ int wave_shr1z(int x) { return __builtin_amdgcn_update_dpp(0, x, 0x138, 0xf, 0xf, true); }
__device__ __forceinline__ int wave_shl1z(int x) { return __builtin_amdgcn_update_dpp(0, x, 0x130, 0xf, 0xf, true); }
__device__ __forceinline__ int wave_shl1(int x, int fill) { return dppi<0x130, 0xf>(fill, x); }

__device__ __forceinline__ int wave_scan_max_self(int x) { return wave_scan_max(x, -0x7fffffff - 1); }

#define RI_KEEP 0x8000u
#define RI_RING 0x10000u
#define RI_CHAIN_MASK ((3u << 3) | (31u << 5) | RI_KEEP)
#define RI_CHAIN_VAL ((1u << 3) | (1u << 5))
#define RI_ONE_MASK ((3u << 3) | RI_KEEP)
#define RI_ONE_VAL (1u << 3)

struct ArrI {
  int32_t* W; uint32_t o;
  __device__ __forceinline__ int32_t& operator[](int i) const { return W[o + (uint32_t)i]; }
};
struct ArrU {
  int32_t* W; uint32_t o;
  __device__ __forceinline__ uint32_t& operator[](int i) const { return ((uint32_t*)W)[o + (uint32_t)i]; }
};

__device__ unsigned long long g_poaw_prof[8];
#ifdef POA_COUNT_ROWS
__device__ unsigned long long g_poaw_rows[16];
#define ROWCNT(k) (++rowcnt[k])
#else
#define ROWCNT(k)
#endif
#define PROF_T() (prof_t = wall_clock64())
#define PROF_ADD(k) do { const unsigned long long t_ = wall_clock64(); prof[k] += t_ - prof_t; prof_t = t_; } while (0)

#ifdef POA_MIN_WAVES
#define POA_BOUNDS __launch_bounds__(64, POA_MIN_WAVES)
#else
#define POA_BOUNDS __launch_bounds__(64)
#endif
template <int C>
__global__ void POA_BOUNDS poa_wave_kernel(const PoaWaveTask* tasks, const uint8_t* seqs, const int64_t* seq_off,
                                                     int32_t* ws32, uint8_t* ws8, int32_t* cons_len, int32_t* status,
                                                     unsigned long long* cells) {
  extern __shared__ __align__(16) unsigned char smem[];
  const PoaWaveTask T = tasks[blockIdx.x];
  const int lane = threadIdx.x;
  const int nc = T.nc, ec = T.ec, WS = T.ws, wm = WS - 1, RS = T.rs, RING = T.ring, rm = RING - 1, NS = RING + 2;
  constexpr int G = 4;
  constexpr bool CHAIN = C <= 2;
  const int RST = RS + 2 * G;
  int32_t* rH = (int32_t*)smem;
  int32_t* rE1 = rH + NS * RST;
  int32_t* rE2 = rE1 + NS * RST;
  int32_t* rbeg = rE2 + NS * RST;
  int32_t* rend = rbeg + NS;
  int32_t* rmpl = rend + NS;
  int32_t* rmpr = rmpl + NS;
  int32_t* sh = rmpr + NS;
  uint8_t* q = (uint8_t*)(sh + 16) + 16;
  const WsLayout wl = ws_layout(nc, ec, T.max_len, WS);
  int32_t* const W = ws32 + T.ws_off;
  const ArrI out_head{W, (uint32_t)wl.out_head}, in_head{W, (uint32_t)wl.in_head}, order{W, (uint32_t)wl.order},
      index{W, (uint32_t)wl.index}, col{W, (uint32_t)wl.col}, base{W, (uint32_t)wl.base}, row_beg{W, (uint32_t)wl.row_beg},
      row_end{W, (uint32_t)wl.row_end}, hl{W, (uint32_t)wl.hl}, row_mpl{W, (uint32_t)wl.row_mpl},
      row_mpr{W, (uint32_t)wl.row_mpr}, aln{W, (uint32_t)wl.aln}, scr{W, (uint32_t)wl.scr}, e_from{W, (uint32_t)wl.e_from},
      e_to{W, (uint32_t)wl.e_to}, e_w{W, (uint32_t)wl.e_w}, e_next_out{W, (uint32_t)wl.e_next_out},
      e_next_in{W, (uint32_t)wl.e_next_in}, op_node{W, (uint32_t)wl.op_node}, op_q{W, (uint32_t)wl.op_q},
      path_use{W, (uint32_t)wl.path_use}, gH{W, (uint32_t)wl.gH}, gE1{W, (uint32_t)wl.gE1}, gE2{W, (uint32_t)wl.gE2};
  const ArrU prow0{W, (uint32_t)wl.prow0}, prow1{W, (uint32_t)wl.prow1}, rinfo{W, (uint32_t)wl.rinfo},
      keepf{W, (uint32_t)wl.keepf}, path_aux{W, (uint32_t)wl.path_aux}, gdir{W, (uint32_t)wl.gdir};
  const int opcap = nc + T.max_len + 4;
  const int n = (int)T.n_seqs;
  unsigned long long my_cells = 0;
  unsigned long long prof[5] = {0, 0, 0, 0, 0}, prof_t;
#ifdef POA_COUNT_ROWS
  unsigned rowcnt[16] = {0};
#endif
#ifdef POA_FINE_PROF
  long long fp[6] = {0, 0, 0, 0, 0, 0}, ft = 0;
#define FP(k) do { const long long t_ = clock64(); fp[k] += t_ - ft; ft = t_; } while (0)
#else
#define FP(k)
#endif
  if (n <= 0) { if (lane == 0) { cons_len[blockIdx.x] = 0; status[blockIdx.x] = 0; } return; }
  if (T.prio >= 3) __builtin_amdgcn_s_setprio(3);
  else if (T.prio == 2) __builtin_amdgcn_s_setprio(2);
  else if (T.prio == 1) __builtin_amdgcn_s_setprio(1);
#define FAIL(code) do { status[blockIdx.x] = (code); return; } while (0)
  {
    const uint8_t* q0 = seqs + seq_off[T.seq_first];
    const int L0 = (int)(seq_off[T.seq_first + 1] - seq_off[T.seq_first]);
    if (L0 + 2 > nc || L0 + 1 > ec) FAIL(3 | (1 << 8));
    for (int v = lane; v < L0 + 2; v += 64) {
      const int b = v < 2 ? 4 : q0[v - 2];
      base[v] = b;
      out_head[v] = v == 1 ? -1 : (v == 0 ? 0 : v - 1);
      in_head[v] = v == 0 ? -1 : (v == 1 ? L0 : v - 2);
      for (int x = 0; x < 5; ++x) aln[5 * v + x] = -1;
      if (v >= 2) aln[5 * v + b] = v;
      const int idx = v == 0 ? 0 : v == 1 ? L0 + 1 : v - 1;
      col[v] = v == 1 ? COL_SINK : idx;
      index[v] = idx;
      order[idx] = v;
    }
    for (int e = lane; e <= L0; e += 64) {
      e_from[e] = e == 0 ? 0 : e + 1;
      e_to[e] = e == L0 ? 1 : e + 2;
      e_w[e] = 1;
      e_next_out[e] = -1; e_next_in[e] = -1;
    }
    if (lane == 0) { sh[0] = L0 + 2; sh[1] = L0 + 1; sh[2] = L0 + 1; }
    __syncthreads();
  }
  for (int i = 1; i < n; ++i) {
    const uint8_t* qg = seqs + seq_off[T.seq_first + i];
    const int L = UNI((int)(seq_off[T.seq_first + i + 1] - seq_off[T.seq_first + i]));
    const int N = __builtin_amdgcn_readfirstlane(sh[0]);
    if (L > T.max_len) FAIL(3 | (6 << 8));
    PROF_T();
    for (int j = lane; j < L; j += 64) q[j] = qg[j];
    if (lane == 0) q[-1] = 4;
    for (int r = lane; r < N + 64; r += 64) {
      uint32_t ri = 0;
      if (r < N) {
        const int v = order[r];
        ri = (uint32_t)base[v] & 7u;
        int np = 0, d0 = 0, d1 = 0;
        for (int e = in_head[v]; e >= 0; e = e_next_in[e]) {
          const int d = r - index[e_from[e]];
          if (np == 0) d0 = d; else if (np == 1) d1 = d;
          ++np;
        }
        if (np > 2 || d0 > 31 || d1 > 31) ri |= RI_SLOW << 3;
        else {
          ri |= ((uint32_t)np << 3) | ((uint32_t)d0 << 5) | ((uint32_t)d1 << 10);
          prow0[r] = (uint32_t)d0 | ((uint32_t)d1 << 8);
          prow1[r] = 0;
        }
        hl[r] = PNEG;
      }
      rinfo[r] = ri;
      keepf[r] = 0;
    }
    __syncthreads();
    auto flag_row = [&](int rr, int d) { if (d >= 2) atomicOr(&keepf[rr], d >= RING ? RI_KEEP : RI_RING); };
    for (int r = lane; r < N - 1; r += 64) {
      const uint32_t ri = rinfo[r];
      const uint32_t np = (ri >> 3) & 3u;
      if (np == RI_SLOW) {
        for (int e = in_head[order[r]]; e >= 0; e = e_next_in[e]) {
          const int d = r - index[e_from[e]];
          flag_row(r - d, d);
        }
      } else {
        const int d0 = (int)((ri >> 5) & 31u), d1 = (int)((ri >> 10) & 31u);
        if (np >= 1) flag_row(r - d0, d0);
        if (np >= 2) flag_row(r - d1, d1);
      }
    }
    __syncthreads();
    PROF_ADD(0);
    int nops = -1;
    for (int attempt = 0; attempt < 2 && nops < 0; ++attempt) {
      const int w = UNI(attempt ? L : 10 + (int)(0.01 * L));
      int last_r = -1, last_mpl = 0, last_mpr = 0, last_beg = 0, last_end = 0;
      auto stage = [&](int ur, int s) {
        __syncthreads();
        const int pb = __builtin_amdgcn_readfirstlane(row_beg[ur]), pe = __builtin_amdgcn_readfirstlane(row_end[ur]);
        const int po = ur * WS;
        for (int x = lane; x <= pe - pb; x += 64) {
          const int o = po + ((pb + x) & wm);
          rH[s * RST + G + x] = gH[o]; rE1[s * RST + G + x] = gE1[o]; rE2[s * RST + G + x] = gE2[o];
        }
        if (lane < G) {
          const int o1 = s * RST + lane, o2 = s * RST + G + (pe - pb + 1) + lane;
          rH[o1] = PNEG; rE1[o1] = PNEG; rE2[o1] = PNEG;
          rH[o2] = PNEG; rE1[o2] = PNEG; rE2[o2] = PNEG;
        }
        if (lane == 0) { rbeg[s] = pb; rend[s] = pe; rmpl[s] = row_mpl[ur]; rmpr[s] = row_mpr[ur]; }
        __syncthreads();
      };
      uint32_t ri_blk = 0;
      int blk0 = -64;
      for (int r_ = 0; r_ < N - 1; ++r_) {
        int r = UNI(r_);
        last_r = UNI(last_r); last_mpl = UNI(last_mpl); last_mpr = UNI(last_mpr); last_beg = UNI(last_beg); last_end = UNI(last_end);
        blk0 = UNI(blk0);
        FP(5);
        if (r - blk0 >= 64) {
          blk0 = r;
          ri_blk = rinfo[r + lane] | keepf[r + lane];
          asm volatile("" : "+v"(ri_blk));
        }
        uint32_t ri = __builtin_amdgcn_readlane(ri_blk, r - blk0);
        if (CHAIN && 64 * C <= WS && r > 0 && (ri & RI_ONE_MASK) == RI_ONE_VAL && (int)((ri >> 5) & 31u) < RING &&
            ((ri >> 5) & 31u) >= 1u && (((ri >> 5) & 31u) != 1u || last_r == r - 1)) {
#ifdef POA_COUNT_ROWS
          const unsigned long long chain_t0 = wall_clock64();
#endif
          int pbeg = 0, pend = 0, pm_l = 0, pm_r = 0;
          int32_t pH[C], pE1[C], pE2[C];
          bool in_ring = true;
          int qc[C], qx[C];
          auto load_pred = [&](int ur) {
            const int sl = ur & rm;
            if (ur == last_r) { pbeg = last_beg; pend = last_end; pm_l = last_mpl; pm_r = last_mpr; }
            else { pbeg = UNI(rbeg[sl]); pend = UNI(rend[sl]); pm_l = UNI(rmpl[sl]); pm_r = UNI(rmpr[sl]); }
            const int so = sl * RST + G;
#pragma unroll
            for (int c = 0; c < C; ++c) {
              const int idx = lane * C + c;
              const bool ok = idx <= pend - pbeg;
              const int a = so + (ok ? idx : 0);
              const int32_t x0 = rH[a], x1 = rE1[a], x2 = rE2[a];
              pH[c] = ok ? tg_up(x0, TG_M) : 0; pE1[c] = ok ? tg_up(x1, TG_E1) : 0; pE2[c] = ok ? tg_up(x2, TG_E2) : 0;
            }
            const int jb = pbeg + lane * C;
#pragma unroll
            for (int c = 0; c < C; ++c) { qc[c] = q[imin(jb + c, L) - 1]; qx[c] = q[imin(jb + c, L - 1)]; }
            in_ring = true;
          };
          load_pred(r - (int)((ri >> 5) & 31u));
          auto ring_store = [&](int rr_, int b_, int e_, const int32_t* h_, const int32_t* e1_, const int32_t* e2_, int l_, int r_) {
            const int sl = rr_ & rm, sb_ = sl * RST + G;
#pragma unroll
            for (int c = 0; c < C; ++c) {
              const int idx = lane * C + c;
              if (idx <= e_ - b_) { rH[sb_ + idx] = tg_down(h_[c]); rE1[sb_ + idx] = tg_down(e1_[c]); rE2[sb_ + idx] = tg_down(e2_[c]); }
            }
            if (lane < G) {
              const int o1 = sl * RST + lane, o2 = sb_ + (e_ - b_ + 1) + lane;
              rH[o1] = PNEG; rE1[o1] = PNEG; rE2[o1] = PNEG;
              rH[o2] = PNEG; rE1[o2] = PNEG; rE2[o2] = PNEG;
            }
            if (lane == 0) { rbeg[sl] = b_; rend[sl] = e_; rmpl[sl] = l_; rmpr[sl] = r_; }
          };
          for (;;) {
            int beg = pm_l + 1 - w; if (beg < 0) beg = 0;
            int end = pm_r + 1 + w; if (end > L) end = L;
            if (end - beg + 1 > 2 * w + 129) end = beg + 2 * w + 128;
            const int width = end - beg + 1;
            const int delta = beg - pbeg;
            if (width > 64 * C || width > RS || (unsigned)delta > 1u) break;
            if (__builtin_expect(delta == 0, 0)) {
              if (pend - pbeg + 1 >= 64 * C) break;
              const int32_t tH = wave_shr1z(pH[C - 1]), t1 = wave_shr1z(pE1[C - 1]), t2 = wave_shr1z(pE2[C - 1]);
#pragma unroll
              for (int c = C - 1; c > 0; --c) { pH[c] = pH[c - 1]; pE1[c] = pE1[c - 1]; pE2[c] = pE2[c - 1]; }
              pH[0] = tH; pE1[0] = t1; pE2[0] = t2;
#pragma unroll
              for (int c = 0; c < C; ++c) qx[c] = qc[c];
            }
            my_cells += (unsigned long long)width;
            ROWCNT(1);
            const int bv = (int)(ri & 7u);
            const int s_mat = bv < 4 ? P_MATCH * TG : 0, s_mis = bv < 4 ? -P_MISMATCH * TG : 0;
            const int jb = beg + lane * C;
            const int32_t nH = wave_shl1z(pH[0]), n1 = wave_shl1z(pE1[0]), n2 = wave_shl1z(pE2[0]);
            int32_t m0[C], e1[C], e2[C], hp[C], hq[C], t1[C], t2[C], p1[C], p2[C];
            uint32_t dw[C];
            bool valid[C];
#pragma unroll
            for (int c = 0; c < C; ++c) {
              const int j = jb + c;
              valid[c] = j <= end;
              const int32_t hA = pH[c], hB = c + 1 < C ? pH[c + 1] : nH, xa = c + 1 < C ? pE1[c + 1] : n1, xb = c + 1 < C ? pE2[c + 1] : n2;
              qc[c] = qx[c];
              int sc = qc[c] == bv ? s_mat : s_mis;
              sc = qc[c] >= 4 ? 0 : sc;
              m0[c] = hA + sc;
              const int32_t a1 = hB - (P_O1 + P_E1) * TG - (TG_M - TG_E1), b1 = xa - P_E1 * TG;
              const int32_t a2 = hB - (P_O2 + P_E2) * TG - (TG_M - TG_E2), b2 = xb - P_E2 * TG;
              e1[c] = imax(a1, b1); e2[c] = imax(a2, b2);
              dw[c] = (b1 > a1 ? 0x800u : 0u) | (b2 > a2 ? 0x8000u : 0u);
              hp[c] = valid[c] ? imax(m0[c], imax(e1[c], e2[c])) : 0;
              hq[c] = hp[c] | TG_M;
              t1[c] = hq[c] + j * (P_E1 * TG); t2[c] = hq[c] + j * (P_E2 * TG);
              p1[c] = c ? imax(p1[c - 1], t1[c]) : t1[c];
              p2[c] = c ? imax(p2[c - 1], t2[c]) : t2[c];
            }
#pragma unroll
            for (int c = 0; c < C; ++c) qx[c] = q[imin(jb + c, L - 1)];
            int32_t lmax = hq[0];
#pragma unroll
            for (int c = 1; c < C; ++c) lmax = imax(lmax, hq[c]);
            const int32_t s1 = wave_scan_max_self(p1[C - 1]), s2 = wave_scan_max_self(p2[C - 1]), s3 = wave_scan_max_self(lmax);
            const int32_t X1 = wave_shr1z(s1), X2 = wave_shr1z(s2);
            const int32_t t1_prev = wave_shr1z(t1[C - 1]), t2_prev = wave_shr1z(t2[C - 1]);
            int32_t h[C];
            const int rowo = r * WS;
#pragma unroll
            for (int c = 0; c < C; ++c) {
              const int j = jb + c;
              const int32_t x1 = c ? imax(X1, p1[c - 1]) : X1, x2 = c ? imax(X2, p2[c - 1]) : X2;
              const int32_t f1 = x1 - (P_O1 * TG + (TG_M - TG_F1)) - j * (P_E1 * TG), f2 = x2 - (P_O2 * TG + (TG_M - TG_F2)) - j * (P_E2 * TG);
              h[c] = imax(hp[c], imax(f1, f2));
              const uint32_t dH = ~(uint32_t)h[c] & 15u, dHp = ~(uint32_t)hp[c] & 15u;
              const uint32_t o1 = (c ? t1[c - 1] : t1_prev) == x1 ? 0x10000u : 0u;
              const uint32_t o2 = (c ? t2[c - 1] : t2_prev) == x2 ? 0x20000u : 0u;
              *(uint32_t*)((char*)W + (((gdir.o + (uint32_t)(rowo + (j & wm))) << 2) & 0xfffffffcu)) = dw[c] | dH | (dHp << 4) | o1 | o2;
            }
            if (end == L) {
#pragma unroll
              for (int c = 0; c < C; ++c) if (jb + c == L) hl[r] = tg_down(h[c]);
            }
#pragma unroll
            for (int c = 0; c < C; ++c) { pH[c] = valid[c] ? (h[c] | TG_M) : 0; pE1[c] = valid[c] ? e1[c] : 0; pE2[c] = valid[c] ? e2[c] : 0; }
            const int32_t wmx = __builtin_amdgcn_readlane(s3, 63);
            int l = 1 << 20, rr = -1;
#pragma unroll
            for (int c = 0; c < C; ++c) {
              const unsigned long long em = __ballot(hq[c] == wmx);
              if (em) { l = imin(l, C * (int)__builtin_ctzll(em) + c); rr = imax(rr, C * (63 - (int)__builtin_clzll(em)) + c); }
            }
            l += beg; rr += beg;
            if (wmx <= TGB / 2) { l = beg; rr = end; }
            last_r = r; last_mpl = UNI(l); last_mpr = UNI(rr); last_beg = beg; last_end = end;
            pbeg = beg; pend = end; pm_l = last_mpl; pm_r = last_mpr;
            in_ring = (ri & RI_RING) != 0;
            if (in_ring) ring_store(r, beg, end, pH, pE1, pE2, l, rr);
            ++r;
            if (r >= N - 1) break;
            if (r - blk0 >= 64) {
              blk0 = r;
              ri_blk = rinfo[r + lane] | keepf[r + lane];
              asm volatile("" : "+v"(ri_blk));
            }
            ri = __builtin_amdgcn_readlane(ri_blk, r - blk0);
            if ((ri & RI_ONE_MASK) != RI_ONE_VAL) break;
            const int dn = (int)((ri >> 5) & 31u);
            if (dn != 1) {
              if (dn < 1 || dn >= RING) break;
              ROWCNT(9);
              load_pred(r - dn);
            }
          }
          if (!in_ring) ring_store(r - 1, pbeg, pend, pH, pE1, pE2, last_mpl, last_mpr);
#ifdef POA_COUNT_ROWS
          prof[4] += wall_clock64() - chain_t0;
          ROWCNT(2);
#endif
          if (r >= N - 1) break;
          r_ = r;
        }
        const int slot = r & rm;
        const int bv = (int)(ri & 7u);
        int np = (int)((ri >> 3) & 3u);
        const bool keep = ((ri >> 15) & 1u) != 0;
        const bool slow = np == (int)RI_SLOW;
        int ps0 = 0, ps1 = 0;
        int lo = 1 << 30, hi = -1;
        uint32_t pd0 = 0, pd1 = 0;
        if (!slow) {
          int nfar = 0;
          if (np >= 1) {
            const int d = (int)((ri >> 5) & 31u), ur = r - d;
            pd0 = (uint32_t)imin(d, 255);
            if (d < RING) ps0 = ur & rm; else { ps0 = RING + nfar++; stage(ur, ps0); }
            const int a = ur == last_r ? last_mpl : __builtin_amdgcn_readfirstlane(rmpl[ps0]);
            const int b = ur == last_r ? last_mpr : __builtin_amdgcn_readfirstlane(rmpr[ps0]);
            lo = imin(lo, a); hi = imax(hi, b);
          }
          if (np >= 2) {
            const int d = (int)((ri >> 10) & 31u), ur = r - d;
            pd0 |= (uint32_t)imin(d, 255) << 8;
            if (d < RING) ps1 = ur & rm; else { ps1 = RING + nfar++; stage(ur, ps1); }
            const int a = ur == last_r ? last_mpl : __builtin_amdgcn_readfirstlane(rmpl[ps1]);
            const int b = ur == last_r ? last_mpr : __builtin_amdgcn_readfirstlane(rmpr[ps1]);
            lo = imin(lo, a); hi = imax(hi, b);
          }
        } else {
          int nfar = 0;
          np = 0;
          for (int e = __builtin_amdgcn_readfirstlane(in_head[order[r]]); e >= 0; e = __builtin_amdgcn_readfirstlane(e_next_in[e])) {
            const int ur = __builtin_amdgcn_readfirstlane(index[e_from[e]]);
            if (np < 8) {
              const uint32_t dl = (uint32_t)imin(r - ur, 255);
              if (np < 4) pd0 |= dl << (8 * np); else pd1 |= dl << (8 * (np - 4));
              int s;
              if (r - ur < RING) s = ur & rm;
              else {
                if (nfar >= 2) FAIL(3 | (2 << 8));
                s = RING + nfar++;
                stage(ur, s);
              }
              sh[8 + np] = s;
              const int a = ur == last_r ? last_mpl : __builtin_amdgcn_readfirstlane(rmpl[s]);
              const int b = ur == last_r ? last_mpr : __builtin_amdgcn_readfirstlane(rmpr[s]);
              lo = imin(lo, a); hi = imax(hi, b);
            }
            ++np;
          }
          if (np > 8) FAIL(3 | (2 << 8));
        }
        int beg, end;
        if (r == 0) { beg = 0; end = w < L ? w : L; }
        else {
          beg = lo + 1 - w; if (beg < 0) beg = 0;
          end = hi + 1 + w; if (end > L) end = L;
          if (end - beg + 1 > 2 * w + 129) end = beg + 2 * w + 128;
        }
        const int width = end - beg + 1;
        if (width > RS || width > WS) FAIL(3 | (3 << 8));
        my_cells += (unsigned long long)width;
        if (lane == 0) {
          rbeg[slot] = beg; rend[slot] = end;
          prow0[r] = pd0; prow1[r] = pd1;
          if (end < L) hl[r] = PNEG;
          if (keep) { row_beg[r] = beg; row_end[r] = end; }
        }
        FP(0);
        const int rowo = r * WS;
        const int sb = slot * RST + G;
        if (lane < G) {
          const int o1 = slot * RST + lane, o2 = sb + width + lane;
          rH[o1] = PNEG; rE1[o1] = PNEG; rE2[o1] = PNEG;
          rH[o2] = PNEG; rE1[o2] = PNEG; rE2[o2] = PNEG;
        }
        int pb0 = 0, pb1 = 0;
        bool fast = !slow && np >= 1;
        if (fast) {
          int pe0;
          if (np == 1 && (int)(pd0 & 255u) == 1 && last_r == r - 1) { pb0 = last_beg; pe0 = last_end; }
          else { pb0 = __builtin_amdgcn_readfirstlane(rbeg[ps0]); pe0 = __builtin_amdgcn_readfirstlane(rend[ps0]); }
          fast = beg - 1 >= pb0 - G && end <= pe0 + G;
          if (np == 2) {
            pb1 = __builtin_amdgcn_readfirstlane(rbeg[ps1]);
            fast = fast && beg - 1 >= pb1 - G && end <= __builtin_amdgcn_readfirstlane(rend[ps1]) + G;
          }
        }
        const int this_beg = beg, this_end = end;
#ifdef POA_COUNT_ROWS
        ROWCNT(7);
        if (slow) ROWCNT(4); else if (!fast) ROWCNT(3); else if (np == 2) ROWCNT(15);
        else if (C == 1 && !keep && width <= 64) ROWCNT(0); else ROWCNT(14);
        if (!slow && np == 1 && (pd0 & 255u) == 1 && !keep) { ROWCNT(5); if (width <= 64 * C) ROWCNT(8); if (last_beg == beg - 1) ROWCNT(9); if (last_beg == beg) ROWCNT(10); }
        if (!slow && np == 2 && ((pd0 & 255u) == 1 || ((pd0 >> 8) & 255u) == 1) && fast && !keep) ROWCNT(6);
        if (!slow && np == 1 && (pd0 & 255u) > 1 && fast && !keep) ROWCNT(11);
        if (keep) ROWCNT(12);
        if (width <= 64) ROWCNT(13);
#endif
        if (C == 1 && fast && np == 1 && !keep && width <= 64) {
          const int j = beg + lane;
          const bool valid = j <= end;
          const int scv = (j >= 1 && valid) ? pl_score(bv, q[j - 1]) : 0;
          const int bi0 = ps0 * RST + G + (j - 1 - pb0);
          const int32_t hvA = rH[bi0], hvB = rH[bi0 + 1], xa = rE1[bi0 + 1], xb = rE2[bi0 + 1];
          const int32_t m0 = hvA + scv;
          const int32_t a1 = hvB - P_O1 - P_E1, b1 = xa - P_E1;
          const int32_t e1v = imax(a1, b1);
          const uint32_t dE1v = a1 == e1v ? 0u : 8u;
          const int32_t a2 = hvB - P_O2 - P_E2, b2 = xb - P_E2;
          const int32_t e2v = imax(a2, b2);
          const uint32_t dE2v = a2 == e2v ? 0u : 8u;
          const int32_t hpv = valid ? imax(m0, imax(e1v, e2v)) : PNEG;
          const int32_t s1 = wave_scan_max(hpv + j * P_E1, PNEG), s2 = wave_scan_max(hpv + j * P_E2, PNEG), s3 = wave_scan_max(hpv, PNEG);
          const int32_t f1 = wave_shr1(s1, PNEG) - P_O1 - j * P_E1, f2 = wave_shr1(s2, PNEG) - P_O2 - j * P_E2;
          const int32_t h = imax(hpv, imax(f1, f2));
          const int32_t hp_left = wave_shr1(hpv, PNEG);
          if (valid) {
            const uint32_t dH = m0 == h ? 0u : e1v == h ? 8u : e2v == h ? 9u : f1 == h ? 10u : 11u;
            const uint32_t dHp = m0 == hpv ? 0u : e1v == hpv ? 8u : 9u;
            const uint32_t o1 = hp_left - P_O1 - P_E1 == f1 ? 1u : 0u;
            const uint32_t o2 = hp_left - P_O2 - P_E2 == f2 ? 1u : 0u;
            gdir[rowo + (j & wm)] = dH | (dHp << 4) | (dE1v << 8) | (dE2v << 12) | (o1 << 16) | (o2 << 17);
            rH[sb + lane] = h; rE1[sb + lane] = e1v; rE2[sb + lane] = e2v;
            if (j == L) hl[r] = h;
          }
          const int32_t wmx = __builtin_amdgcn_readlane(s3, 63);
          const unsigned long long em = __ballot(valid && hpv == wmx);
          int l = beg + (int)__builtin_ctzll(em), rr = beg + 63 - (int)__builtin_clzll(em);
          if (wmx <= PNEG / 2) { l = beg; rr = end; }
          last_r = r; last_mpl = UNI(l); last_mpr = UNI(rr); last_beg = this_beg; last_end = this_end;
          if (lane == 0) { rmpl[slot] = l; rmpr[slot] = rr; }
          continue;
        }
        int32_t lbest = -0x7fffffff - 1; int ll = -1, lr = -1;
        int32_t g1 = PNEG, g2 = PNEG, hpc = PNEG;
        for (int j0 = beg; j0 <= end; j0 += 64 * C) {
          const int jb = j0 + lane * C;
          int32_t m[C], e1[C], e2[C];
          int km[C];
          uint32_t dE1[C], dE2[C];
          int sc[C];
#pragma unroll
          for (int c = 0; c < C; ++c) {
            const int j = jb + c;
            sc[c] = (j >= 1 && j <= end) ? pl_score(bv, q[j - 1]) : 0;
          }
          if (fast) {
            int32_t hv0[C + 1], xa0[C], xb0[C];
            const int bi0 = ps0 * RST + G + (jb - 1 - pb0);
#pragma unroll
            for (int t = 0; t <= C; ++t) hv0[t] = rH[bi0 + t];
#pragma unroll
            for (int t = 0; t < C; ++t) { xa0[t] = rE1[bi0 + 1 + t]; xb0[t] = rE2[bi0 + 1 + t]; }
            if (np == 1) {
#pragma unroll
              for (int c = 0; c < C; ++c) {
                m[c] = hv0[c] + sc[c]; km[c] = 0;
                const int32_t a1 = hv0[c + 1] - P_O1 - P_E1, b1 = xa0[c] - P_E1;
                e1[c] = imax(a1, b1); dE1[c] = a1 == e1[c] ? 0u : 8u;
                const int32_t a2 = hv0[c + 1] - P_O2 - P_E2, b2 = xb0[c] - P_E2;
                e2[c] = imax(a2, b2); dE2[c] = a2 == e2[c] ? 0u : 8u;
              }
            } else {
              int32_t hv1[C + 1], xa1[C], xb1[C];
              const int bi1 = ps1 * RST + G + (jb - 1 - pb1);
#pragma unroll
              for (int t = 0; t <= C; ++t) hv1[t] = rH[bi1 + t];
#pragma unroll
              for (int t = 0; t < C; ++t) { xa1[t] = rE1[bi1 + 1 + t]; xb1[t] = rE2[bi1 + 1 + t]; }
#pragma unroll
              for (int c = 0; c < C; ++c) {
                const int32_t m0 = hv0[c] + sc[c], m1 = hv1[c] + sc[c];
                m[c] = imax(m0, m1); km[c] = m1 > m0 ? 1 : 0;
                {
                  const int32_t a0 = hv0[c + 1] - P_O1 - P_E1, b0 = xa0[c] - P_E1, a1 = hv1[c + 1] - P_O1 - P_E1, b1 = xa1[c] - P_E1;
                  const int32_t e = imax(imax(a0, b0), imax(a1, b1));
                  e1[c] = e; dE1[c] = a0 == e ? 0u : a1 == e ? 1u : b0 == e ? 8u : 9u;
                }
                {
                  const int32_t a0 = hv0[c + 1] - P_O2 - P_E2, b0 = xb0[c] - P_E2, a1 = hv1[c + 1] - P_O2 - P_E2, b1 = xb1[c] - P_E2;
                  const int32_t e = imax(imax(a0, b0), imax(a1, b1));
                  e2[c] = e; dE2[c] = a0 == e ? 0u : a1 == e ? 1u : b0 == e ? 8u : 9u;
                }
              }
            }
          } else {
            int ko1[C], kx1[C], ko2[C], kx2[C];
#pragma unroll
            for (int c = 0; c < C; ++c) {
              m[c] = PNEG; e1[c] = PNEG; e2[c] = PNEG;
              km[c] = 15; ko1[c] = 15; kx1[c] = 15; ko2[c] = 15; kx2[c] = 15;
            }
            auto accum = [&](int k, int sl) {
              const int pb = __builtin_amdgcn_readfirstlane(rbeg[sl]), pe = __builtin_amdgcn_readfirstlane(rend[sl]);
              const int so = sl * RST + G;
              int32_t hv[C + 1], x1v[C], x2v[C];
#pragma unroll
              for (int t = 0; t <= C; ++t) {
                const int jj = jb - 1 + t;
                const bool ok = jj >= pb && jj <= pe && jj <= end;
                const int32_t val = rH[so + (ok ? jj - pb : 0)];
                hv[t] = ok ? val : PNEG;
              }
#pragma unroll
              for (int t = 0; t < C; ++t) {
                const int jj = jb + t;
                const bool ok = jj >= pb && jj <= pe && jj <= end;
                const int32_t v1 = rE1[so + (ok ? jj - pb : 0)], v2 = rE2[so + (ok ? jj - pb : 0)];
                x1v[t] = ok ? v1 : PNEG;
                x2v[t] = ok ? v2 : PNEG;
              }
#pragma unroll
              for (int c = 0; c < C; ++c) {
                const int32_t hm1 = hv[c], h = hv[c + 1];
                if (hm1 > PNEG / 2) { const int32_t x = hm1 + sc[c]; if (x > m[c]) { m[c] = x; km[c] = k; } }
                {
                  const int32_t a = h > PNEG / 2 ? h - P_O1 - P_E1 : PNEG, b = x1v[c] > PNEG / 2 ? x1v[c] - P_E1 : PNEG;
                  const int32_t cc = a > b ? a : b;
                  if (cc > PNEG / 2) {
                    if (cc > e1[c]) { e1[c] = cc; ko1[c] = 15; kx1[c] = 15; }
                    if (cc == e1[c]) { if (a == cc && ko1[c] == 15) ko1[c] = k; if (b == cc && kx1[c] == 15) kx1[c] = k; }
                  }
                }
                {
                  const int32_t a = h > PNEG / 2 ? h - P_O2 - P_E2 : PNEG, b = x2v[c] > PNEG / 2 ? x2v[c] - P_E2 : PNEG;
                  const int32_t cc = a > b ? a : b;
                  if (cc > PNEG / 2) {
                    if (cc > e2[c]) { e2[c] = cc; ko2[c] = 15; kx2[c] = 15; }
                    if (cc == e2[c]) { if (a == cc && ko2[c] == 15) ko2[c] = k; if (b == cc && kx2[c] == 15) kx2[c] = k; }
                  }
                }
              }
            };
            if (r == 0) {
#pragma unroll
              for (int c = 0; c < C; ++c) if (jb + c == 0) m[c] = 0;
            } else if (!slow) {
              if (np >= 1) accum(0, ps0);
              if (np >= 2) accum(1, ps1);
            } else {
#pragma unroll 1
              for (int k = 0; k < np; ++k) accum(k, __builtin_amdgcn_readfirstlane(sh[8 + k]));
            }
#pragma unroll
            for (int c = 0; c < C; ++c) {
              dE1[c] = ko1[c] != 15 ? (uint32_t)ko1[c] : (uint32_t)(8 + (kx1[c] & 7));
              dE2[c] = ko2[c] != 15 ? (uint32_t)ko2[c] : (uint32_t)(8 + (kx2[c] & 7));
            }
          }
          FP(1);
          int32_t hp[C], p1[C], p2[C];
#pragma unroll
          for (int c = 0; c < C; ++c) {
            const int j = jb + c;
            int32_t x = imax(m[c], imax(e1[c], e2[c]));
            if (j > end) x = PNEG;
            hp[c] = x;
            const int32_t t1 = x + j * P_E1, t2 = x + j * P_E2;
            p1[c] = c ? imax(p1[c - 1], t1) : t1;
            p2[c] = c ? imax(p2[c - 1], t2) : t2;
          }
          const int32_t s1 = wave_scan_max(p1[C - 1], PNEG), s2 = wave_scan_max(p2[C - 1], PNEG);
          const int32_t X1 = imax(wave_shr1(s1, PNEG), g1), X2 = imax(wave_shr1(s2, PNEG), g2);
          g1 = imax(g1, __builtin_amdgcn_readlane(s1, 63));
          g2 = imax(g2, __builtin_amdgcn_readlane(s2, 63));
          FP(2);
          int32_t hp_prev = wave_shr1(hp[C - 1], PNEG);
          if (lane == 0) hp_prev = hpc;
          hpc = __builtin_amdgcn_readlane(hp[C - 1], 63);
#pragma unroll
          for (int c = 0; c < C; ++c) {
            const int j = jb + c;
            const int32_t x1 = c ? imax(X1, p1[c - 1]) : X1, x2 = c ? imax(X2, p2[c - 1]) : X2;
            const int32_t f1 = x1 - P_O1 - j * P_E1, f2 = x2 - P_O2 - j * P_E2;
            const int32_t h = imax(hp[c], imax(f1, f2));
            const int32_t hp_left = c ? hp[c - 1] : hp_prev;
            if (j <= end) {
              const bool mk = km[c] != 15;
              const uint32_t dH = (m[c] == h && mk) ? (uint32_t)km[c] : e1[c] == h ? 8u : e2[c] == h ? 9u : f1 == h ? 10u : 11u;
              const uint32_t dHp = (m[c] == hp[c] && mk) ? (uint32_t)km[c] : e1[c] == hp[c] ? 8u : 9u;
              const uint32_t o1 = hp_left - P_O1 - P_E1 == f1 ? 1u : 0u;
              const uint32_t o2 = hp_left - P_O2 - P_E2 == f2 ? 1u : 0u;
              const int o = rowo + (j & wm);
              gdir[o] = dH | (dHp << 4) | (dE1[c] << 8) | (dE2[c] << 12) | (o1 << 16) | (o2 << 17);
              if (keep) { gH[o] = h; gE1[o] = e1[c]; gE2[o] = e2[c]; }
              rH[sb + (j - beg)] = h; rE1[sb + (j - beg)] = e1[c]; rE2[sb + (j - beg)] = e2[c];
              if (j == L) hl[r] = h;
              if (h > lbest) { lbest = h; ll = j; lr = j; }
              else if (h == lbest) lr = j;
            }
          }
        }
        FP(3);
        {
          const bool own = ll >= 0;
          const int32_t wmx = __builtin_amdgcn_readlane(wave_scan_max(own ? lbest : -0x7fffffff - 1, -0x7fffffff - 1), 63);
          const bool eq = own && lbest == wmx;
          int l, rr;
          if (width <= 64 * C) {
            const unsigned long long em = __ballot(eq);
            l = __builtin_amdgcn_readlane(ll, (int)__builtin_ctzll(em));
            rr = __builtin_amdgcn_readlane(lr, 63 - (int)__builtin_clzll(em));
          } else {
            l = __builtin_amdgcn_readlane(wave_scan_min(eq ? ll : 0x7fffffff, 0x7fffffff), 63);
            rr = __builtin_amdgcn_readlane(wave_scan_max(eq ? lr : -1, -1), 63);
          }
          if (wmx <= PNEG / 2) { l = beg; rr = end; }
          last_r = r; last_mpl = UNI(l); last_mpr = UNI(rr); last_beg = this_beg; last_end = this_end;
          if (lane == 0) {
            rmpl[slot] = l; rmpr[slot] = rr;
            if (keep) { row_mpl[r] = l; row_mpr[r] = rr; }
          }
        }
        FP(4);
      }
      __syncthreads();
      PROF_ADD(1);
      {
        int bu = -1; int32_t bsc = PNEG;
        for (int e = in_head[1]; e >= 0; e = e_next_in[e]) {
          const int ur = index[e_from[e]];
          const int32_t h = hl[ur];
          if (h > bsc) { bsc = h; bu = ur; }
        }
        nops = -1;
        if (bu >= 0 && bsc > PNEG / 2) {
          nops = 0;
          int r = __builtin_amdgcn_readfirstlane(bu), j = L, st = 0;
          int r0 = -(1 << 28), j0 = 0;
          uint32_t W0 = 0, W1 = 0, W2 = 0, W3 = 0, P0 = 0, P1 = 0;
          while (r != 0 || j > 0) {
            r = UNI(r); j = UNI(j); st = UNI(st); nops = UNI(nops); r0 = UNI(r0); j0 = UNI(j0);
            if (nops + j + 2 > opcap) { nops = -1; break; }
            if (r == 0) {
              for (int t = lane; t < j; t += 64) { op_node[nops + t] = -1; op_q[nops + t] = j - 1 - t; }
              nops += j; j = 0;
              break;
            }
            int k = r0 - r, d = k - (j0 - j);
            if (k < 0 || k > 63 || d < 0 || d > 3) {
              r0 = r; j0 = j; k = 0; d = 0;
              const int rr = r0 - lane;
              if (rr >= 0) {
                const int bp = rr * WS;
                const int c = j0 - lane;
                W0 = gdir[bp + (c & wm)]; W1 = gdir[bp + ((c + 1) & wm)]; W2 = gdir[bp + ((c + 2) & wm)];
                W3 = gdir[bp + ((c + 3) & wm)];
                P0 = prow0[rr]; P1 = prow1[rr];
              }
              asm volatile("" : "+v"(W0), "+v"(W1), "+v"(W2), "+v"(W3), "+v"(P0), "+v"(P1));
            }
            const uint32_t wsel = d == 0 ? W0 : d == 1 ? W1 : d == 2 ? W2 : W3;
            if (st == 0) {
              const bool diag = (wsel & 15u) == 0u && (P0 & 255u) == 1u && r0 - lane >= 1;
              const unsigned long long dm = __ballot(diag) >> k;
              int run = dm == ~0ull ? 64 : (int)__builtin_ctzll(~dm);
              if (run > j) run = j;
              if (run > 0) {
                if (lane < run) { op_node[nops + lane] = r - lane; op_q[nops + lane] = j - 1 - lane; }
                nops += run; r -= run; j -= run;
                continue;
              }
            }
            const uint32_t dw = __builtin_amdgcn_readlane(wsel, k);
            const uint32_t p0 = __builtin_amdgcn_readlane(P0, k), p1 = __builtin_amdgcn_readlane(P1, k);
            int s = -1;
            if (st == 0 || st == 5) {
              const uint32_t dd = st == 0 ? (dw & 15u) : ((dw >> 4) & 15u);
              if (dd < 8) {
                if (lane == 0) { op_node[nops] = r; op_q[nops] = j - 1; }
                ++nops; --j; st = 0; s = (int)dd;
              } else st = (int)dd - 7;
            } else if (st == 1 || st == 2) {
              const uint32_t dd = st == 1 ? ((dw >> 8) & 15u) : ((dw >> 12) & 15u);
              if (lane == 0) { op_node[nops] = r; op_q[nops] = -1; }
              ++nops; s = (int)(dd & 7u);
              if (dd < 8) st = 0;
            } else {
              const uint32_t open = st == 3 ? ((dw >> 16) & 1u) : ((dw >> 17) & 1u);
              if (lane == 0) { op_node[nops] = -1; op_q[nops] = j - 1; }
              ++nops;
              if (open) st = 5;
              --j;
            }
            if (s >= 0) {
              const uint32_t dl = ((s < 4 ? p0 : p1) >> (8 * (s & 3))) & 255u;
              if (dl != 255u) r -= (int)dl;
              else {
                int e = in_head[order[r]];
                for (int t = 0; t < s; ++t) e = e_next_in[e];
                r = __builtin_amdgcn_readfirstlane(index[e_from[e]]);
              }
            }
          }
        }
      }
      __syncthreads();
      PROF_ADD(2);
    }
    if (nops < 0) FAIL(3 | (4 << 8));
    if (nops > 32000) FAIL(3 | (5 << 8));
    const int ncols = __builtin_amdgcn_readfirstlane(sh[2]), n_old = N;
    for (int c = lane; c < ncols; c += 64) scr[c] = 0;
    __syncthreads();
    int carry_c = 0, carry_n = 0, carry_key = 0;
    for (int p0 = 0; p0 < nops; p0 += 64) {
      const int p = p0 + lane;
      const bool valid = p < nops;
      int row = -1, j = -1;
      if (valid) { row = op_node[nops - 1 - p]; j = op_q[nops - 1 - p]; }
      const bool ali = valid && row >= 0 && j >= 0, ins = valid && row < 0;
      const int v = ali ? order[row] : -1;
      const int qb = (ali || ins) ? (int)q[j] : 0;
      int use = -1;
      bool isnew = ins;
      if (ali) {
        if (base[v] == qb) use = v;
        else { const int a = aln[5 * v + qb]; if (a >= 0) use = a; else isnew = true; }
      }
      const int inc_c = wave_scan_add((ali || ins) ? 1 : 0), inc_n = wave_scan_add(isnew ? 1 : 0);
      const int cidx = carry_c + inc_c - ((ali || ins) ? 1 : 0);
      const int nrank = carry_n + inc_n - (isnew ? 1 : 0);
      const int key = ali ? (((cidx + 1) << 16) | col[v]) : 0;
      const int inc_k = wave_scan_max(key, 0);
      const int ikey = imax(carry_key, inc_k);
      carry_c += __builtin_amdgcn_readlane(inc_c, 63);
      carry_n += __builtin_amdgcn_readlane(inc_n, 63);
      carry_key = imax(carry_key, __builtin_amdgcn_readlane(inc_k, 63));
      uint32_t aux = 0xFFFFFFFFu;
      if (isnew && n_old + nrank < nc) {
        const int nid = n_old + nrank;
        use = nid;
        base[nid] = qb;
        out_head[nid] = -1; in_head[nid] = -1;
        if (ali) {
          for (int b = 0; b < 5; ++b) {
            const int sib = aln[5 * v + b];
            aln[5 * nid + b] = sib;
            if (sib >= 0) aln[5 * sib + qb] = nid;
          }
          aln[5 * nid + qb] = nid;
          col[nid] = col[v];
        } else {
          for (int b = 0; b < 5; ++b) aln[5 * nid + b] = b == qb ? nid : -1;
          col[nid] = COL_NEW;
          const int ac = ikey & 0xffff, t = (cidx + 1) - (ikey >> 16);
          atomicMax(&scr[ac], t);
          aux = (uint32_t)ac | ((uint32_t)t << 16);
        }
      }
      if (ali || ins) { path_use[cidx] = use; path_aux[cidx] = aux; }
    }
    const int PC = carry_c, n_new = n_old + carry_n;
    if (n_new > nc || ncols + carry_n > nc || ncols + carry_n > 65000 || PC > 65000) FAIL(3 | (5 << 8));
    __syncthreads();
    for (int t = lane; t <= PC; t += 64) {
      const int u = t == 0 ? 0 : path_use[t - 1], v = t == PC ? 1 : path_use[t];
      int tail = -1, e = out_head[u];
      bool found = false;
      for (; e >= 0; e = e_next_out[e]) {
        if (e_to[e] == v) { e_w[e]++; found = true; break; }
        tail = e;
      }
      if (found) continue;
      const int ne = atomicAdd(&sh[1], 1);
      if (ne >= ec) continue;
      e_from[ne] = u; e_to[ne] = v; e_w[ne] = 1;
      e_next_out[ne] = -1; e_next_in[ne] = -1;
      if (tail < 0) out_head[u] = ne; else e_next_out[tail] = ne;
      int ie = in_head[v];
      if (ie < 0) in_head[v] = ne;
      else {
        while (e_next_in[ie] >= 0) ie = e_next_in[ie];
        e_next_in[ie] = ne;
      }
    }
    __syncthreads();
    if (sh[1] > ec) FAIL(3 | (5 << 8));
    int carry = 0;
    for (int c0 = 0; c0 < ncols; c0 += 64) {
      const int c = c0 + lane;
      const int x = c < ncols ? scr[c] : 0;
      const int inc = wave_scan_add(x);
      if (c < ncols) scr[c] = carry + inc - x;
      carry += __builtin_amdgcn_readlane(inc, 63);
    }
    __syncthreads();
    for (int v = lane; v < n_new; v += 64) {
      const int cv = col[v];
      if (cv < COL_SINK) col[v] = cv + scr[cv];
    }
    __syncthreads();
    for (int t = lane; t < PC; t += 64) {
      const uint32_t aux = path_aux[t];
      if (aux != 0xFFFFFFFFu) { const int ac = (int)(aux & 0xffffu); col[path_use[t]] = ac + scr[ac] + (int)(aux >> 16); }
    }
    const int ncols_new = ncols + carry;
    __syncthreads();
    for (int c = lane; c < ncols_new; c += 64) scr[c] = 0;
    __syncthreads();
    for (int v = lane; v < n_new; v += 64) if (v != 1) atomicAdd(&scr[col[v]], 1);
    __syncthreads();
    carry = 0;
    for (int c0 = 0; c0 < ncols_new; c0 += 64) {
      const int c = c0 + lane;
      const int x = c < ncols_new ? scr[c] : 0;
      const int inc = wave_scan_add(x);
      if (c < ncols_new) scr[c] = carry + inc - x;
      carry += __builtin_amdgcn_readlane(inc, 63);
    }
    __syncthreads();
    for (int v = lane; v < n_new; v += 64) if (v != 1) {
      const int pos = atomicAdd(&scr[col[v]], 1);
      order[pos] = v; index[v] = pos;
    }
    if (lane == 0) { order[n_new - 1] = 1; index[1] = n_new - 1; sh[0] = n_new; sh[2] = ncols_new; }
    __syncthreads();
    PROF_ADD(3);
  }
  if (lane == 0) {
    cons_len[blockIdx.x] = sh[0];
    status[blockIdx.x] = 0;
    atomicAdd(cells, my_cells);
    for (int k = 0; k < 5; ++k) atomicAdd(&g_poaw_prof[k], prof[k]);
#ifdef POA_COUNT_ROWS
    for (int k = 0; k < 16; ++k) atomicAdd(&g_poaw_rows[k], (unsigned long long)rowcnt[k]);
#endif
#ifdef POA_FINE_PROF
    for (int k = 0; k < 6; ++k) printf("fp%d %lld\n", k, fp[k]);
#endif
  }
#undef FAIL
}

__global__ void __launch_bounds__(64) poa_bundle_kernel(const PoaWaveTask* tasks, int32_t* ws32, uint8_t* ws8, int32_t* cons_len,
                                                       const int32_t* status) {
  extern __shared__ __align__(16) unsigned char smem[];
  if (status[blockIdx.x] != 0) return;
  const PoaWaveTask T = tasks[blockIdx.x];
  const int lane = threadIdx.x;
  const int nc = T.nc;
  const int N = cons_len[blockIdx.x];
  if (T.n_seqs <= 0 || N <= 0) return;
  const WsLayout wl = ws_layout(nc, T.ec, T.max_len, T.ws);
  int32_t* W = ws32 + T.ws_off;
  const int32_t *out_head = W + wl.out_head, *order = W + wl.order, *index = W + wl.index, *base = W + wl.base;
  const int32_t *e_to = W + wl.e_to, *e_w = W + wl.e_w, *e_next_out = W + wl.e_next_out;
  uint8_t* cons = ws8 + T.cons_off;
  uint32_t* succ0 = (uint32_t*)smem;
  uint32_t* succ1 = succ0 + nc;
  int32_t* score = (int32_t*)(succ1 + nc);
  for (int r = lane; r < N; r += 64) {
    const int v = order[r];
    uint32_t s0 = 0xFFFFu, s1 = 0xFFFFu;
    int k = 0;
    for (int e = out_head[v]; e >= 0; e = e_next_out[e]) {
      const uint32_t ent = (uint32_t)index[e_to[e]] | ((uint32_t)e_w[e] << 16);
      if (k == 0) s0 = ent; else if (k == 1) s1 = ent;
      ++k;
    }
    if (k > 2) s1 = 0xFFFFu | (0x1FFFu << 16);
    succ0[r] = s0 | ((uint32_t)base[v] << 29);
    succ1[r] = s1;
  }
  __syncthreads();
  if (lane == 0) {
    for (int r = N - 1; r >= 0; --r) {
      const uint32_t s0 = succ0[r], s1 = succ1[r];
      int bst = -1, bw = -1; int32_t bsc = -1;
      if ((s1 & 0xFFFFu) == 0xFFFFu && ((s1 >> 16) & 0x1FFFu) == 0x1FFFu) {
        for (int e = out_head[order[r]]; e >= 0; e = e_next_out[e]) {
          const int x = index[e_to[e]], wgt = e_w[e];
          const int32_t sx = score[x];
          if (wgt > bw || (wgt == bw && sx > bsc)) { bw = wgt; bsc = sx; bst = x; }
        }
      } else {
        if ((s0 & 0xFFFFu) != 0xFFFFu) { bst = (int)(s0 & 0xFFFFu); bw = (int)((s0 >> 16) & 0x1FFFu); bsc = score[bst]; }
        if ((s1 & 0xFFFFu) != 0xFFFFu) {
          const int x = (int)(s1 & 0xFFFFu), wgt = (int)((s1 >> 16) & 0x1FFFu);
          const int32_t sx = score[x];
          if (wgt > bw || (wgt == bw && sx > bsc)) { bw = wgt; bsc = sx; bst = x; }
        }
      }
      succ1[r] = (uint32_t)bst;
      score[r] = bst >= 0 ? bw + bsc : 0;
    }
    int len = 0;
    const int sink_row = N - 1;
    for (int r = (int)succ1[0]; r >= 0 && r != sink_row; r = (int)succ1[r]) cons[len++] = (uint8_t)(succ0[r] >> 29);
    cons_len[blockIdx.x] = len;
  }
}

template <int C>
static hipError_t launch_c(const PoaWaveTask* d_tasks, int n_tasks, size_t lds_bytes, const uint8_t* d_seqs,
                           const int64_t* d_seq_off, int32_t* ws32, uint8_t* ws8, int32_t* d_len, int32_t* d_status,
                           unsigned long long* d_cells, hipStream_t stream) {
  hipError_t e = hipFuncSetAttribute((const void*)poa_wave_kernel<C>, hipFuncAttributeMaxDynamicSharedMemorySize, (int)lds_bytes);
  if (e != hipSuccess) return e;
  hipLaunchKernelGGL(poa_wave_kernel<C>, dim3((unsigned)n_tasks), dim3(64), lds_bytes, stream, d_tasks, d_seqs, d_seq_off, ws32, ws8,
                     d_len, d_status, d_cells);
  return hipGetLastError();
}

hipError_t poa_wave_launch(int cols, const PoaWaveTask* d_tasks, int n_tasks, size_t lds_bytes, size_t bundle_lds_bytes,
                           const uint8_t* d_seqs, const int64_t* d_seq_off, int32_t* ws32, uint8_t* ws8, int32_t* d_len,
                           int32_t* d_status, unsigned long long* d_cells, hipStream_t stream) {
  hipError_t e;
  if (cols == 1) e = launch_c<1>(d_tasks, n_tasks, lds_bytes, d_seqs, d_seq_off, ws32, ws8, d_len, d_status, d_cells, stream);
  else if (cols == 2) e = launch_c<2>(d_tasks, n_tasks, lds_bytes, d_seqs, d_seq_off, ws32, ws8, d_len, d_status, d_cells, stream);
  else if (cols == 3) e = launch_c<3>(d_tasks, n_tasks, lds_bytes, d_seqs, d_seq_off, ws32, ws8, d_len, d_status, d_cells, stream);
  else if (cols == 5) e = launch_c<5>(d_tasks, n_tasks, lds_bytes, d_seqs, d_seq_off, ws32, ws8, d_len, d_status, d_cells, stream);
  else return hipErrorInvalidValue;
  if (e != hipSuccess) return e;
  return poa_bundle_launch(d_tasks, n_tasks, bundle_lds_bytes, ws32, ws8, d_len, (const int32_t*)d_status, stream);
}

hipError_t poa_bundle_launch(const PoaWaveTask* d_tasks, int n_tasks, size_t bundle_lds_bytes, int32_t* ws32, uint8_t* ws8, int32_t* d_len,
                             const int32_t* d_status, hipStream_t stream) {
  hipError_t e = hipFuncSetAttribute((const void*)poa_bundle_kernel, hipFuncAttributeMaxDynamicSharedMemorySize, (int)bundle_lds_bytes);
  if (e != hipSuccess) return e;
  hipLaunchKernelGGL(poa_bundle_kernel, dim3((unsigned)n_tasks), dim3(64), bundle_lds_bytes, stream, d_tasks, ws32, ws8, d_len, d_status);
  return hipGetLastError();
}

void poa_wave_debug_report() {
  unsigned long long h[8];
  if (hipMemcpyFromSymbol(h, HIP_SYMBOL(g_poaw_prof), sizeof h) != hipSuccess) return;
  fprintf(stderr, "[poa_wave] 100MHz ticks (sum over clusters): prepare %llu forward %llu traceback %llu update %llu bundle %llu\n",
          h[0], h[1], h[2], h[3], h[4]);
  memset(h, 0, sizeof h);
  (void)hipMemcpyToSymbol(HIP_SYMBOL(g_poaw_prof), h, sizeof h);
#ifdef POA_COUNT_ROWS
  unsigned long long rc[16];
  if (hipMemcpyFromSymbol(rc, HIP_SYMBOL(g_poaw_rows), sizeof rc) != hipSuccess) return;
  fprintf(stderr, "[poa_wave] rows: chain %llu in %llu chains (time: the 'bundle' figure above) | other rows %llu: flat %llu fast1 %llu fast2 %llu general %llu slow %llu | "
          "of them chain-eligible %llu (fits lanes %llu, band +1 %llu, +0 %llu) np2-with-prev %llu np1-far %llu keep %llu width<=64 %llu\n", rc[1], rc[2], rc[7],
          rc[0], rc[14], rc[15], rc[3], rc[4], rc[5], rc[8], rc[9], rc[10], rc[6], rc[11], rc[12], rc[13]);
  memset(rc, 0, sizeof rc);
  (void)hipMemcpyToSymbol(HIP_SYMBOL(g_poaw_rows), rc, sizeof rc);
#endif
}
```

Measured before the change: 8.518 million.

## Stage call-path host transfers through double-buffered pinned memory and cache LDS attributes

Replaces the direct pageable hipMemcpyAsync calls in alignment, LCS ratio and POA with a per-batch double-buffered pinned staging engine. Large copies are split into chunks so the host memcpy of one chunk overlaps the DMA of the other, which avoids the pageable-copy path. Separately, repeated hipFuncSetAttribute calls for dynamic LDS size are cached per kernel and device, so the attribute is only raised when a larger size is needed. The staging adds extra host memcpy work and event synchronisation per chunk, and pinned buffers are kept per thread-local state.

Result: no change. 8.444 million (-0.9%).

```diff
diff --git a/svdss_amd/csrc/call_dp.hip b/svdss_amd/csrc/call_dp.hip
--- a/svdss_amd/csrc/call_dp.hip
+++ b/svdss_amd/csrc/call_dp.hip
@@ -12,7 +12,9 @@
 #include "../../include/svdss_hip.h"
 #include "call_streams.h"
 #include "dev_arena.h"
+#include "dyn_lds.h"
 #include "hip_check.h"
+#include "pin_stage.h"
 
 #define DP_NEG (-0x20000000)
 #define DP_THREADS 256
@@ -342,6 +344,7 @@
   std::vector<uint32_t> cigar;
   int device = -1;
   DevArena arena;
+  CallStage stage;
 };
 
 namespace {
@@ -383,11 +386,13 @@
   const int64_t qtot = q_off[n_pairs] - q_off[0], ttot = t_off[n_pairs] - t_off[0];
   if (b->device != device) {
     b->arena.drop();
+    b->stage.drop();
     b->device = device;
   }
   CallStreamLease lease;
   HIPCHK(lease.acquire(device));
   const hipStream_t st = lease.get();
+  HIPCHK(b->stage.begin());
   const GapModel gm{gapo, gape, gapo2, gape2};
   hipEvent_t ev0, ev1;
   HIPCHK(hipEventCreate(&ev0));
@@ -460,10 +465,10 @@
     void* d_sc = b->arena.take(sizeof(int32_t) * (size_t)np);
     void* d_nc = b->arena.take(sizeof(int32_t) * (size_t)np);
     void* d_abort = b->arena.take(64);
-    if (qtot) HIPCHK(hipMemcpyAsync(d_q, queries + q_off[0], (size_t)qtot, hipMemcpyHostToDevice, st));
-    if (ttot) HIPCHK(hipMemcpyAsync(d_t, targets + t_off[0], (size_t)ttot, hipMemcpyHostToDevice, st));
-    HIPCHK(hipMemcpyAsync(d_mat, mat, (size_t)(m * m), hipMemcpyHostToDevice, st));
-    HIPCHK(hipMemcpyAsync(d_pairs, hp.data(), sizeof(AlnPair) * (size_t)np, hipMemcpyHostToDevice, st));
+    if (qtot) HIPCHK(b->stage.up(d_q, queries + q_off[0], (size_t)qtot, st));
+    if (ttot) HIPCHK(b->stage.up(d_t, targets + t_off[0], (size_t)ttot, st));
+    HIPCHK(b->stage.up(d_mat, mat, (size_t)(m * m), st));
+    HIPCHK(b->stage.up(d_pairs, hp.data(), sizeof(AlnPair) * (size_t)np, st));
     HIPCHK(hipMemsetAsync(d_abort, 0, 64, st));
     HIPCHK(hipEventRecord(ev0, st));
     if (any_multi && ALN_W == 8)
@@ -482,8 +487,9 @@
     HIPCHK(hipEventRecord(ev1, st));
     if (any_multi) {
       int32_t ab = 0;
-      HIPCHK(hipMemcpyAsync(&ab, d_abort, sizeof ab, hipMemcpyDeviceToHost, st));
+      HIPCHK(b->stage.down(&ab, d_abort, sizeof ab, st));
       HIPCHK(hipStreamSynchronize(st));
+      HIPCHK(b->stage.drain());
       if (ab) {
         fprintf(stderr, "[svdss] realignment: a multi-wavefront pair did not finish; the batch runs again with one wavefront per pair\n");
         multi = false;
@@ -497,10 +503,11 @@
     for (const AlnPair& a : hp) b->info[1] += a.waves > 1;
     b->info[2] = std::max<int64_t>(b->info[2], any_multi ? ALN_W : 1);
     chunk_cigs.emplace_back((size_t)cig);
-    HIPCHK(hipMemcpyAsync(&b->scores[(size_t)start], d_sc, sizeof(int32_t) * (size_t)np, hipMemcpyDeviceToHost, st));
-    HIPCHK(hipMemcpyAsync(&h_nc[(size_t)start], d_nc, sizeof(int32_t) * (size_t)np, hipMemcpyDeviceToHost, st));
-    if (cig) HIPCHK(hipMemcpyAsync(chunk_cigs.back().data(), d_cig, sizeof(uint32_t) * (size_t)cig, hipMemcpyDeviceToHost, st));
+    HIPCHK(b->stage.down(&b->scores[(size_t)start], d_sc, sizeof(int32_t) * (size_t)np, st));
+    HIPCHK(b->stage.down(&h_nc[(size_t)start], d_nc, sizeof(int32_t) * (size_t)np, st));
+    if (cig) HIPCHK(b->stage.down(chunk_cigs.back().data(), d_cig, sizeof(uint32_t) * (size_t)cig, st));
     HIPCHK(hipStreamSynchronize(st));
+    HIPCHK(b->stage.drain());
     float ms = 0.f;
     HIPCHK(hipEventElapsedTime(&ms, ev0, ev1));
     b->kernel_ms += ms;
@@ -575,15 +582,18 @@
   struct RatioState {
     int device = -1;
     DevArena arena;
+    CallStage stage;
   };
   static thread_local RatioState R;
   if (R.device != device) {
     R.arena.drop();
+    R.stage.drop();
     R.device = device;
   }
   CallStreamLease lease;
   HIPCHK(lease.acquire(device));
   const hipStream_t st = lease.get();
+  HIPCHK(R.stage.begin());
   HIPCHK(R.arena.reserve(DevArena::padded((size_t)atot) + DevArena::padded((size_t)btot) +
                           DevArena::padded(sizeof(LcsPair) * (size_t)n_pairs) + DevArena::padded(sizeof(int32_t) * (size_t)ws) +
                           DevArena::padded(sizeof(int64_t) * (size_t)n_pairs) + DevArena::padded(sizeof(double) * (size_t)n_pairs) +
@@ -591,9 +601,9 @@
   struct { void* p; } d_a{R.arena.take((size_t)atot)}, d_b{R.arena.take((size_t)btot)},
       d_pairs{R.arena.take(sizeof(LcsPair) * (size_t)n_pairs)}, d_ws{R.arena.take(sizeof(int32_t) * (size_t)ws)},
       d_lcs{R.arena.take(sizeof(int64_t) * (size_t)n_pairs)}, d_ratio{R.arena.take(sizeof(double) * (size_t)n_pairs)};
-  if (atot) HIPCHK(hipMemcpyAsync(d_a.p, a + a_off[0], (size_t)atot, hipMemcpyHostToDevice, st));
-  if (btot) HIPCHK(hipMemcpyAsync(d_b.p, bsy + b_off[0], (size_t)btot, hipMemcpyHostToDevice, st));
-  HIPCHK(hipMemcpyAsync(d_pairs.p, hp.data(), sizeof(LcsPair) * (size_t)n_pairs, hipMemcpyHostToDevice, st));
+  if (atot) HIPCHK(R.stage.up(d_a.p, a + a_off[0], (size_t)atot, st));
+  if (btot) HIPCHK(R.stage.up(d_b.p, bsy + b_off[0], (size_t)btot, st));
+  HIPCHK(R.stage.up(d_pairs.p, hp.data(), sizeof(LcsPair) * (size_t)n_pairs, st));
   bool bits_ok = !getenv("SVDSS_RATIO_DP");
   uint8_t sym_id[256];
   if (bits_ok) {
@@ -616,19 +626,21 @@
   }
   if (bits_ok) {
     void* d_map = R.arena.take(256);
-    HIPCHK(hipMemcpyAsync(d_map, sym_id, 256, hipMemcpyHostToDevice, st));
+    HIPCHK(R.stage.up(d_map, sym_id, 256, st));
     g_ratio_last_kernel = 0;
     hipLaunchKernelGGL(lcs_bits_kernel, dim3((unsigned)n_pairs), dim3(64), 0, st, (const LcsPair*)d_pairs.p,
                        (const uint8_t*)d_a.p, (const uint8_t*)d_b.p, (const uint8_t*)d_map, (int64_t*)d_lcs.p, (double*)d_ratio.p);
     HIPCHK(hipGetLastError());
-    HIPCHK(hipMemcpyAsync(ratio_out, d_ratio.p, sizeof(double) * (size_t)n_pairs, hipMemcpyDeviceToHost, st));
-    if (lcs_out) HIPCHK(hipMemcpyAsync(lcs_out, d_lcs.p, sizeof(int64_t) * (size_t)n_pairs, hipMemcpyDeviceToHost, st));
+    HIPCHK(R.stage.down(ratio_out, d_ratio.p, sizeof(double) * (size_t)n_pairs, st));
+    if (lcs_out) HIPCHK(R.stage.down(lcs_out, d_lcs.p, sizeof(int64_t) * (size_t)n_pairs, st));
     HIPCHK(hipStreamSynchronize(st));
+    HIPCHK(R.stage.drain());
     return SVDSS_OK;
   }
   const size_t lds_need = sizeof(int32_t) * 3 * (size_t)(la_max + 1) + (size_t)la_max + (size_t)lb_max + 16;
   if (lds_need <= 150 * 1024) {
-    HIPCHK(hipFuncSetAttribute((const void*)lcs_ratio_kernel<true>, hipFuncAttributeMaxDynamicSharedMemorySize, (int)lds_need));
+    static DynLdsMax lds_max;
+    HIPCHK(lds_max.need((const void*)lcs_ratio_kernel<true>, device, lds_need));
     g_ratio_last_kernel = 1;
     hipLaunchKernelGGL(lcs_ratio_kernel<true>, dim3((unsigned)n_pairs), dim3(DP_THREADS), lds_need, st,
                        (const LcsPair*)d_pairs.p, (const uint8_t*)d_a.p, (const uint8_t*)d_b.p, (int32_t*)d_ws.p,
@@ -640,8 +652,9 @@
                        (int64_t*)d_lcs.p, (double*)d_ratio.p);
   }
   HIPCHK(hipGetLastError());
-  HIPCHK(hipMemcpyAsync(ratio_out, d_ratio.p, sizeof(double) * (size_t)n_pairs, hipMemcpyDeviceToHost, st));
-  if (lcs_out) HIPCHK(hipMemcpyAsync(lcs_out, d_lcs.p, sizeof(int64_t) * (size_t)n_pairs, hipMemcpyDeviceToHost, st));
+  HIPCHK(R.stage.down(ratio_out, d_ratio.p, sizeof(double) * (size_t)n_pairs, st));
+  if (lcs_out) HIPCHK(R.stage.down(lcs_out, d_lcs.p, sizeof(int64_t) * (size_t)n_pairs, st));
   HIPCHK(hipStreamSynchronize(st));
+  HIPCHK(R.stage.drain());
   return SVDSS_OK;
 }
diff --git a/svdss_amd/csrc/dyn_lds.h b/svdss_amd/csrc/dyn_lds.h
--- /dev/null
+++ b/svdss_amd/csrc/dyn_lds.h
@@ -0,0 +1,24 @@
+#pragma once
+#include <hip/hip_runtime.h>
+
+#include <atomic>
+#include <mutex>
+
+struct DynLdsMax {
+  static constexpr int kDevices = 64;
+  std::atomic<int> have[kDevices];
+  std::mutex mu;
+  DynLdsMax() { for (auto& h : have) h.store(0, std::memory_order_relaxed); }
+
+  hipError_t need(const void* kernel, int device, size_t bytes) {
+    if (device < 0 || device >= kDevices) return hipErrorInvalidDevice;
+    if (bytes > (size_t)0x7fffffff) return hipErrorInvalidValue;
+    const int want = (int)bytes;
+    if (want <= have[device].load(std::memory_order_acquire)) return hipSuccess;
+    std::lock_guard<std::mutex> lock(mu);
+    if (want <= have[device].load(std::memory_order_relaxed)) return hipSuccess;
+    const hipError_t e = hipFuncSetAttribute(kernel, hipFuncAttributeMaxDynamicSharedMemorySize, want);
+    if (e == hipSuccess) have[device].store(want, std::memory_order_release);
+    return e;
+  }
+};
diff --git a/svdss_amd/csrc/pin_stage.h b/svdss_amd/csrc/pin_stage.h
--- /dev/null
+++ b/svdss_amd/csrc/pin_stage.h
@@ -0,0 +1,144 @@
+#pragma once
+#include <cstddef>
+#include <cstdint>
+#include <cstdlib>
+#include <cstring>
+
+inline size_t call_stage_chunk_bytes() {
+  static const size_t bytes = [] {
+    const char* e = getenv("SVDSS_CALL_STAGE_KB");
+    if (!e) return (size_t)4096 << 10;
+    const long long kb = atoll(e);
+    return kb <= 0 ? (size_t)0 : (size_t)(kb > (1 << 20) ? (1 << 20) : kb) << 10;
+  }();
+  return bytes;
+}
+
+template <class Engine>
+class PinStager {
+ public:
+  using Stream = typename Engine::Stream;
+  Engine eng;
+
+  int begin(size_t chunk_bytes) {
+    chunk_ = chunk_bytes;
+    pend_[0].n = pend_[1].n = 0;
+    return chunk_ ? eng.ensure(chunk_) : 0;
+  }
+
+  int up(void* dst, const void* src, size_t n, Stream st) {
+    if (!chunk_) return n ? eng.direct_up(dst, src, n, st) : 0;
+    for (size_t off = 0; off < n; off += chunk_) {
+      const size_t len = n - off < chunk_ ? n - off : chunk_;
+      const int k = (int)(seq_++ & 1);
+      if (const int rc = claim(k)) return rc;
+      memcpy(eng.buf(k), (const char*)src + off, len);
+      if (const int rc = eng.issue_up((char*)dst + off, k, len, st)) return rc;
+    }
+    return 0;
+  }
+
+  int down(void* dst, const void* src, size_t n, Stream st) {
+    if (!chunk_) return n ? eng.direct_down(dst, src, n, st) : 0;
+    for (size_t off = 0; off < n; off += chunk_) {
+      const size_t len = n - off < chunk_ ? n - off : chunk_;
+      const int k = (int)(seq_++ & 1);
+      if (const int rc = claim(k)) return rc;
+      if (const int rc = eng.issue_down(k, (const char*)src + off, len, st)) return rc;
+      pend_[k].dst = (char*)dst + off;
+      pend_[k].n = len;
+    }
+    return 0;
+  }
+
+  int drain() {
+    const int first = (int)(seq_ & 1);
+    if (const int rc = claim(first)) return rc;
+    return claim(first ^ 1);
+  }
+
+ private:
+  int claim(int k) {
+    if (const int rc = eng.wait(k)) return rc;
+    if (pend_[k].n) {
+      memcpy(pend_[k].dst, eng.buf(k), pend_[k].n);
+      pend_[k].n = 0;
+    }
+    return 0;
+  }
+
+  struct Pending { char* dst = nullptr; size_t n = 0; };
+  size_t chunk_ = 0;
+  unsigned seq_ = 0;
+  Pending pend_[2];
+};
+
+#ifdef __HIPCC__
+#include <hip/hip_runtime.h>
+
+struct HipPinEngine {
+  using Stream = hipStream_t;
+  char* b[2] = {nullptr, nullptr};
+  hipEvent_t ev[2] = {nullptr, nullptr};
+  bool flying[2] = {false, false};
+  size_t cap = 0;
+
+  HipPinEngine() = default;
+  HipPinEngine(const HipPinEngine&) = delete;
+  HipPinEngine& operator=(const HipPinEngine&) = delete;
+  ~HipPinEngine() { drop(); }
+
+  void drop() {
+    for (int k = 0; k < 2; ++k) {
+      if (flying[k]) (void)hipEventSynchronize(ev[k]);
+      if (b[k]) (void)hipHostFree(b[k]);
+      if (ev[k]) (void)hipEventDestroy(ev[k]);
+      b[k] = nullptr; ev[k] = nullptr; flying[k] = false;
+    }
+    cap = 0;
+  }
+  int ensure(size_t chunk) {
+    if (chunk <= cap) return 0;
+    drop();
+    for (int k = 0; k < 2; ++k) {
+      hipError_t e = hipHostMalloc((void**)&b[k], chunk, hipHostMallocDefault);
+      if (e == hipSuccess) e = hipEventCreateWithFlags(&ev[k], hipEventDisableTiming);
+      if (e != hipSuccess) { drop(); return (int)e; }
+    }
+    cap = chunk;
+    return 0;
+  }
+  char* buf(int k) { return b[k]; }
+  int issue_up(void* dst, int k, size_t n, hipStream_t st) {
+    const hipError_t e = hipMemcpyAsync(dst, b[k], n, hipMemcpyHostToDevice, st);
+    return e != hipSuccess ? (int)e : mark(k, st);
+  }
+  int issue_down(int k, const void* src, size_t n, hipStream_t st) {
+    const hipError_t e = hipMemcpyAsync(b[k], src, n, hipMemcpyDeviceToHost, st);
+    return e != hipSuccess ? (int)e : mark(k, st);
+  }
+  int wait(int k) {
+    if (!flying[k]) return 0;
+    flying[k] = false;
+    return (int)hipEventSynchronize(ev[k]);
+  }
+  int direct_up(void* dst, const void* src, size_t n, hipStream_t st) { return (int)hipMemcpyAsync(dst, src, n, hipMemcpyHostToDevice, st); }
+  int direct_down(void* dst, const void* src, size_t n, hipStream_t st) { return (int)hipMemcpyAsync(dst, src, n, hipMemcpyDeviceToHost, st); }
+
+ private:
+  int mark(int k, hipStream_t st) {
+    const hipError_t e = hipEventRecord(ev[k], st);
+    flying[k] = e == hipSuccess;
+    return (int)e;
+  }
+};
+
+struct CallStage {
+  PinStager<HipPinEngine> s;
+  hipError_t begin() { return (hipError_t)s.begin(call_stage_chunk_bytes()); }
+  hipError_t up(void* dst, const void* src, size_t n, hipStream_t st) { return (hipError_t)s.up(dst, src, n, st); }
+  hipError_t down(void* dst, const void* src, size_t n, hipStream_t st) { return (hipError_t)s.down(dst, src, n, st); }
+  hipError_t drain() { return (hipError_t)s.drain(); }
+  void drop() { s.eng.drop(); }
+};
+#endif
diff --git a/svdss_amd/csrc/poa.hip b/svdss_amd/csrc/poa.hip
--- a/svdss_amd/csrc/poa.hip
+++ b/svdss_amd/csrc/poa.hip
@@ -14,6 +14,7 @@
 #include "call_streams.h"
 #include "dev_arena.h"
 #include "hip_check.h"
+#include "pin_stage.h"
 #include "poa_plan.h"
 #include "poa_wave.h"
 #include "poa_quad.h"
@@ -358,6 +359,7 @@
   std::vector<uint8_t> cons;
   int device = -1;
   DevArena in_arena, ws_arena;
+  CallStage stage;
 };
 
 static_assert(poa_padded(0) == DevArena::padded(0) && poa_padded(1001) == DevArena::padded(1001), "poa_plan.h sizes what ws_arena hands out");
@@ -402,7 +404,7 @@
     }
     if (total_syms > 0 && !seqs) return SVDSS_EINVAL;
     if (b.device != device) {
-      b.in_arena.drop(); b.ws_arena.drop();
+      b.in_arena.drop(); b.ws_arena.drop(); b.stage.drop();
       b.device = device;
     }
     const size_t off_bytes = sizeof(int64_t) * (size_t)(n_seqs_total + 1);
@@ -410,8 +412,9 @@
     d_seqs = b.in_arena.take((size_t)total_syms); d_off = b.in_arena.take(off_bytes); d_cells = b.in_arena.take(8);
     HIPCHK(lease.acquire(device));
     s0 = lease.get();
-    if (total_syms) HIPCHK(hipMemcpyAsync(d_seqs, seqs, (size_t)total_syms, hipMemcpyHostToDevice, s0));
-    HIPCHK(hipMemcpyAsync(d_off, in.seq_off, off_bytes, hipMemcpyHostToDevice, s0));
+    HIPCHK(b.stage.begin());
+    HIPCHK(b.stage.up(d_seqs, seqs, (size_t)total_syms, s0));
+    HIPCHK(b.stage.up(d_off, in.seq_off, off_bytes, s0));
     HIPCHK(hipMemsetAsync(d_cells, 0, 8, s0));
     hipDeviceProp_t prop;
     if (hipGetDeviceProperties(&prop, device) == hipSuccess && prop.multiProcessorCount > 0) in.n_cus = prop.multiProcessorCount;
@@ -478,7 +481,7 @@
       if (u.pair) u.g = &u.merged;
       const size_t nt = u.g->tasks.size();
       u.m = take(sizeof(PoaWaveTask), nt, u.g->w32, 0, u.g->w8);
-      HIPCHK(hipMemcpyAsync(u.m.tasks, u.g->tasks.data(), sizeof(PoaWaveTask) * nt, hipMemcpyHostToDevice, s0));
+      HIPCHK(b.stage.up(u.m.tasks, u.g->tasks.data(), sizeof(PoaWaveTask) * nt, s0));
       HIPCHK(hipMemsetAsync(u.m.st, 0xff, sizeof(int32_t) * nt, s0));
     }
     std::vector<CallStreamLease> side(units.empty() ? 0 : std::min<size_t>(units.size() - 1, 5));
@@ -495,16 +498,16 @@
       const int nt = (int)g.tasks.size();
       if (u.pair) {
         HIPCHK(poa_quad_pair_launch(d_tasks, (int)u.n2, nt - (int)u.n2, u.max_len2, u.max_len1, (const uint8_t*)d_seqs, (const int64_t*)d_off,
-                                     (int32_t*)m.w32, (int32_t*)m.len, (int32_t*)m.st, (unsigned long long*)d_cells, gs));
-        HIPCHK(poa_bundle_launch(d_tasks, nt, g.bundle_lds, (int32_t*)m.w32, (uint8_t*)m.w8, (int32_t*)m.len, (const int32_t*)m.st, gs));
+                                     (int32_t*)m.w32, (int32_t*)m.len, (int32_t*)m.st, (unsigned long long*)d_cells, gs, b.device));
+        HIPCHK(poa_bundle_launch(d_tasks, nt, g.bundle_lds, (int32_t*)m.w32, (uint8_t*)m.w8, (int32_t*)m.len, (const int32_t*)m.st, gs, b.device));
         if (u.n2 && (size_t)nt > u.n2) { std::lock_guard<std::mutex> lock(call_stream_pool().mu); ++call_stream_pool().merged; }
       } else if (g.gw) {
         HIPCHK(poa_quad_launch(g.gw, g.cols, d_tasks, nt, g.max_len, (const uint8_t*)d_seqs, (const int64_t*)d_off, (int32_t*)m.w32,
-                                (int32_t*)m.len, (int32_t*)m.st, (unsigned long long*)d_cells, gs));
-        HIPCHK(poa_bundle_launch(d_tasks, nt, g.bundle_lds, (int32_t*)m.w32, (uint8_t*)m.w8, (int32_t*)m.len, (const int32_t*)m.st, gs));
+                                (int32_t*)m.len, (int32_t*)m.st, (unsigned long long*)d_cells, gs, b.device));
+        HIPCHK(poa_bundle_launch(d_tasks, nt, g.bundle_lds, (int32_t*)m.w32, (uint8_t*)m.w8, (int32_t*)m.len, (const int32_t*)m.st, gs, b.device));
       } else
         HIPCHK(poa_wave_launch(g.cols, d_tasks, nt, g.lds, g.bundle_lds, (const uint8_t*)d_seqs, (const int64_t*)d_off, (int32_t*)m.w32,
-                                (uint8_t*)m.w8, (int32_t*)m.len, (int32_t*)m.st, (unsigned long long*)d_cells, gs));
+                                (uint8_t*)m.w8, (int32_t*)m.len, (int32_t*)m.st, (unsigned long long*)d_cells, gs, b.device));
     }
     for (CallStreamLease& l : side) HIPCHK(hipStreamSynchronize(l.get()));
     HIPCHK(hipStreamSynchronize(s0));
@@ -530,10 +533,11 @@
     const size_t nt = tasks.size();
     std::vector<int32_t> lens(nt), st(nt);
     std::vector<uint8_t> h8((size_t)w8);
-    HIPCHK(hipMemcpyAsync(lens.data(), m.len, sizeof(int32_t) * nt, hipMemcpyDeviceToHost, s0));
-    HIPCHK(hipMemcpyAsync(st.data(), m.st, sizeof(int32_t) * nt, hipMemcpyDeviceToHost, s0));
-    if (w8) HIPCHK(hipMemcpyAsync(h8.data(), m.w8, (size_t)w8, hipMemcpyDeviceToHost, s0));
+    HIPCHK(b.stage.down(lens.data(), m.len, sizeof(int32_t) * nt, s0));
+    HIPCHK(b.stage.down(st.data(), m.st, sizeof(int32_t) * nt, s0));
+    HIPCHK(b.stage.down(h8.data(), m.w8, (size_t)w8, s0));
     HIPCHK(hipStreamSynchronize(s0));
+    HIPCHK(b.stage.drain());
     for (size_t k = 0; k < nt; ++k) {
       const int64_t id = ids[k];
       if (st[k] == 0) {
@@ -565,7 +569,7 @@
         HIPCHK(b.ws_arena.reserve(poa_padded(sizeof(PoaTask) * nt) + poa_padded(sizeof(int32_t) * (size_t)L.w32) + poa_padded(sizeof(int64_t) * (size_t)L.w64) +
                                   poa_padded((size_t)L.w8) + 2 * poa_padded(sizeof(int32_t) * nt)));
         const Mem m = take(sizeof(PoaTask), nt, L.w32, L.w64, L.w8);
-        HIPCHK(hipMemcpyAsync(m.tasks, L.tasks.data(), sizeof(PoaTask) * nt, hipMemcpyHostToDevice, s0));
+        HIPCHK(b.stage.up(m.tasks, L.tasks.data(), sizeof(PoaTask) * nt, s0));
         HIPCHK(hipMemsetAsync(m.st, 0xff, sizeof(int32_t) * nt, s0));
         if (const int rc = ev.create()) return rc;
         HIPCHK(hipEventRecord(ev.a, s0));
@@ -588,8 +592,9 @@
 
   int gather() {
     unsigned long long cells = 0;
-    HIPCHK(hipMemcpyAsync(&cells, d_cells, 8, hipMemcpyDeviceToHost, s0));
+    HIPCHK(b.stage.down(&cells, d_cells, 8, s0));
     HIPCHK(hipStreamSynchronize(s0));
+    HIPCHK(b.stage.drain());
     b.cells = (int64_t)cells;
     for (int64_t c = 0; c < in.n_clusters; ++c) {
       b.cons_len[(size_t)c] = (int64_t)results[(size_t)c].size();
diff --git a/svdss_amd/csrc/poa_quad.h b/svdss_amd/csrc/poa_quad.h
--- a/svdss_amd/csrc/poa_quad.h
+++ b/svdss_amd/csrc/poa_quad.h
@@ -7,8 +7,8 @@
 #include "poa_task.h"
 
 hipError_t poa_quad_launch(int gw, int cols, const PoaWaveTask* d_tasks, int n_tasks, int max_len, const uint8_t* d_seqs, const int64_t* d_seq_off,
-                           int32_t* ws32, int32_t* d_len, int32_t* d_status, unsigned long long* d_cells, hipStream_t stream);
+                           int32_t* ws32, int32_t* d_len, int32_t* d_status, unsigned long long* d_cells, hipStream_t stream, int device);
 hipError_t poa_quad_pair_launch(const PoaWaveTask* d_tasks, int n2, int n1, int max_len2, int max_len1, const uint8_t* d_seqs,
                                 const int64_t* d_seq_off, int32_t* ws32, int32_t* d_len, int32_t* d_status, unsigned long long* d_cells,
-                                hipStream_t stream);
+                                hipStream_t stream, int device);
 void poa_quad_debug_report();
diff --git a/svdss_amd/csrc/poa_quad.hip b/svdss_amd/csrc/poa_quad.hip
--- a/svdss_amd/csrc/poa_quad.hip
+++ b/svdss_amd/csrc/poa_quad.hip
@@ -5,6 +5,7 @@
 #include <cstdio>
 #include <cstring>
 
+#include "dyn_lds.h"
 #include "poa_plan.h"
 #include "poa_quad.h"
 #include "poa_quad_gfx950.h"
@@ -22,11 +23,12 @@
 
 template <int GW, int C>
 static hipError_t launch_gc(const PoaWaveTask* d_tasks, int n_tasks, int max_len, const uint8_t* d_seqs, const int64_t* d_seq_off, int32_t* ws32,
-                            int32_t* d_len, int32_t* d_status, unsigned long long* d_cells, hipStream_t stream) {
+                            int32_t* d_len, int32_t* d_status, unsigned long long* d_cells, hipStream_t stream, int device) {
   constexpr int G = 64 / GW;
   const size_t lds = pq::Geom<GW, C>::lds_bytes(max_len);
   if (lds > 160 * 1024 - 512) return hipErrorInvalidValue;
-  hipError_t e = hipFuncSetAttribute((const void*)poa_quad_kernel<GW, C>, hipFuncAttributeMaxDynamicSharedMemorySize, (int)lds);
+  static DynLdsMax lds_max;
+  hipError_t e = lds_max.need((const void*)poa_quad_kernel<GW, C>, device, lds);
   if (e != hipSuccess) return e;
   hipLaunchKernelGGL((poa_quad_kernel<GW, C>), dim3((unsigned)((n_tasks + G - 1) / G)), dim3(64), lds, stream, d_tasks, n_tasks, d_seqs,
                      d_seq_off, ws32, d_len, d_status, d_cells, pq::Geom<GW, C>::qcap(max_len));
@@ -44,13 +46,14 @@
 
 hipError_t poa_quad_pair_launch(const PoaWaveTask* d_tasks, int n2, int n1, int max_len2, int max_len1, const uint8_t* d_seqs,
                                 const int64_t* d_seq_off, int32_t* ws32, int32_t* d_len, int32_t* d_status, unsigned long long* d_cells,
-                                hipStream_t stream) {
+                                hipStream_t stream, int device) {
   if (n2 < 0 || n1 < 0 || n2 + n1 <= 0) return hipErrorInvalidValue;
   size_t lds = 0;
   if (n2) lds = std::max(lds, pq::Geom<64, 2>::lds_bytes(max_len2));
   if (n1) lds = std::max(lds, pq::Geom<64, 1>::lds_bytes(max_len1));
   if (lds > 160 * 1024 - 512) return hipErrorInvalidValue;
-  hipError_t e = hipFuncSetAttribute((const void*)poa_quad_pair_kernel, hipFuncAttributeMaxDynamicSharedMemorySize, (int)lds);
+  static DynLdsMax lds_max;
+  hipError_t e = lds_max.need((const void*)poa_quad_pair_kernel, device, lds);
   if (e != hipSuccess) return e;
   hipLaunchKernelGGL(poa_quad_pair_kernel, dim3((unsigned)(n2 + n1)), dim3(64), lds, stream, d_tasks, n2, n1, d_seqs, d_seq_off, ws32, d_len,
                      d_status, d_cells, pq::Geom<64, 2>::qcap(max_len2), pq::Geom<64, 1>::qcap(max_len1));
@@ -58,9 +61,9 @@
 }
 
 hipError_t poa_quad_launch(int gw, int cols, const PoaWaveTask* d_tasks, int n_tasks, int max_len, const uint8_t* d_seqs, const int64_t* d_seq_off,
-                           int32_t* ws32, int32_t* d_len, int32_t* d_status, unsigned long long* d_cells, hipStream_t stream) {
+                           int32_t* ws32, int32_t* d_len, int32_t* d_status, unsigned long long* d_cells, hipStream_t stream, int device) {
 #define PQ_CASE(GW_, C_) \
-  if (gw == GW_ && cols == C_) return launch_gc<GW_, C_>(d_tasks, n_tasks, max_len, d_seqs, d_seq_off, ws32, d_len, d_status, d_cells, stream)
+  if (gw == GW_ && cols == C_) return launch_gc<GW_, C_>(d_tasks, n_tasks, max_len, d_seqs, d_seq_off, ws32, d_len, d_status, d_cells, stream, device)
   PQ_CASE(16, 3); PQ_CASE(16, 4); PQ_CASE(16, 5); PQ_CASE(16, 6); PQ_CASE(16, 7);
   PQ_CASE(32, 2); PQ_CASE(32, 3); PQ_CASE(32, 4);
   PQ_CASE(64, 1); PQ_CASE(64, 2);
diff --git a/svdss_amd/csrc/poa_wave.h b/svdss_amd/csrc/poa_wave.h
--- a/svdss_amd/csrc/poa_wave.h
+++ b/svdss_amd/csrc/poa_wave.h
@@ -8,7 +8,7 @@
 
 hipError_t poa_wave_launch(int cols, const PoaWaveTask* d_tasks, int n_tasks, size_t lds_bytes, size_t bundle_lds_bytes,
                            const uint8_t* d_seqs, const int64_t* d_seq_off, int32_t* ws32, uint8_t* ws8, int32_t* d_len,
-                           int32_t* d_status, unsigned long long* d_cells, hipStream_t stream);
+                           int32_t* d_status, unsigned long long* d_cells, hipStream_t stream, int device);
 hipError_t poa_bundle_launch(const PoaWaveTask* d_tasks, int n_tasks, size_t bundle_lds_bytes, int32_t* ws32, uint8_t* ws8, int32_t* d_len,
-                             const int32_t* d_status, hipStream_t stream);
+                             const int32_t* d_status, hipStream_t stream, int device);
 void poa_wave_debug_report();
diff --git a/svdss_amd/csrc/poa_wave.hip b/svdss_amd/csrc/poa_wave.hip
--- a/svdss_amd/csrc/poa_wave.hip
+++ b/svdss_amd/csrc/poa_wave.hip
@@ -5,6 +5,7 @@
 #include <cstdlib>
 #include <cstring>
 
+#include "dyn_lds.h"
 #include "poa_plan.h"
 #include "poa_wave.h"
 
@@ -1006,8 +1007,9 @@
 template <int C>
 static hipError_t launch_c(const PoaWaveTask* d_tasks, int n_tasks, size_t lds_bytes, const uint8_t* d_seqs,
                            const int64_t* d_seq_off, int32_t* ws32, uint8_t* ws8, int32_t* d_len, int32_t* d_status,
-                           unsigned long long* d_cells, hipStream_t stream) {
-  hipError_t e = hipFuncSetAttribute((const void*)poa_wave_kernel<C>, hipFuncAttributeMaxDynamicSharedMemorySize, (int)lds_bytes);
+                           unsigned long long* d_cells, hipStream_t stream, int device) {
+  static DynLdsMax lds_max;
+  hipError_t e = lds_max.need((const void*)poa_wave_kernel<C>, device, lds_bytes);
   if (e != hipSuccess) return e;
   hipLaunchKernelGGL(poa_wave_kernel<C>, dim3((unsigned)n_tasks), dim3(64), lds_bytes, stream, d_tasks, d_seqs, d_seq_off, ws32, ws8,
                      d_len, d_status, d_cells);
@@ -1016,20 +1018,21 @@
 
 hipError_t poa_wave_launch(int cols, const PoaWaveTask* d_tasks, int n_tasks, size_t lds_bytes, size_t bundle_lds_bytes,
                            const uint8_t* d_seqs, const int64_t* d_seq_off, int32_t* ws32, uint8_t* ws8, int32_t* d_len,
-                           int32_t* d_status, unsigned long long* d_cells, hipStream_t stream) {
+                           int32_t* d_status, unsigned long long* d_cells, hipStream_t stream, int device) {
   hipError_t e;
-  if (cols == 1) e = launch_c<1>(d_tasks, n_tasks, lds_bytes, d_seqs, d_seq_off, ws32, ws8, d_len, d_status, d_cells, stream);
-  else if (cols == 2) e = launch_c<2>(d_tasks, n_tasks, lds_bytes, d_seqs, d_seq_off, ws32, ws8, d_len, d_status, d_cells, stream);
-  else if (cols == 3) e = launch_c<3>(d_tasks, n_tasks, lds_bytes, d_seqs, d_seq_off, ws32, ws8, d_len, d_status, d_cells, stream);
-  else if (cols == 5) e = launch_c<5>(d_tasks, n_tasks, lds_bytes, d_seqs, d_seq_off, ws32, ws8, d_len, d_status, d_cells, stream);
+  if (cols == 1) e = launch_c<1>(d_tasks, n_tasks, lds_bytes, d_seqs, d_seq_off, ws32, ws8, d_len, d_status, d_cells, stream, device);
+  else if (cols == 2) e = launch_c<2>(d_tasks, n_tasks, lds_bytes, d_seqs, d_seq_off, ws32, ws8, d_len, d_status, d_cells, stream, device);
+  else if (cols == 3) e = launch_c<3>(d_tasks, n_tasks, lds_bytes, d_seqs, d_seq_off, ws32, ws8, d_len, d_status, d_cells, stream, device);
+  else if (cols == 5) e = launch_c<5>(d_tasks, n_tasks, lds_bytes, d_seqs, d_seq_off, ws32, ws8, d_len, d_status, d_cells, stream, device);
   else return hipErrorInvalidValue;
   if (e != hipSuccess) return e;
-  return poa_bundle_launch(d_tasks, n_tasks, bundle_lds_bytes, ws32, ws8, d_len, (const int32_t*)d_status, stream);
+  return poa_bundle_launch(d_tasks, n_tasks, bundle_lds_bytes, ws32, ws8, d_len, (const int32_t*)d_status, stream, device);
 }
 
 hipError_t poa_bundle_launch(const PoaWaveTask* d_tasks, int n_tasks, size_t bundle_lds_bytes, int32_t* ws32, uint8_t* ws8, int32_t* d_len,
-                             const int32_t* d_status, hipStream_t stream) {
-  hipError_t e = hipFuncSetAttribute((const void*)poa_bundle_kernel, hipFuncAttributeMaxDynamicSharedMemorySize, (int)bundle_lds_bytes);
+                             const int32_t* d_status, hipStream_t stream, int device) {
+  static DynLdsMax lds_max;
+  hipError_t e = lds_max.need((const void*)poa_bundle_kernel, device, bundle_lds_bytes);
   if (e != hipSuccess) return e;
   hipLaunchKernelGGL(poa_bundle_kernel, dim3((unsigned)n_tasks), dim3(64), bundle_lds_bytes, stream, d_tasks, ws32, ws8, d_len, d_status);
   return hipGetLastError();
```
